# vainaviv/hulk-keypoints

Measured on AMD Instinct MI355X. Metric: images/sec (640x480, N keypoints) inference+train at 1/2/4/8 MI355X, higher is better.
Workload: dtype f32 (f16x3 split-precision MFMA, fp32-accurate); 1 GPU; C2 inference: resnet34-8s K=4 640x480 f16x3 batch 32/GPU (train-mode BN, fused K-ch head, heatmap + argmax, keypoints all-gathered at N>1); mode=infer, backbone=resnet34, keypoints=4, height=480, width=640, batch_per_gpu=32, global_batch=32, parallelism=dp1, bn=per-rank, collectives=none, input=fp32 NCHW (ToTensor)

## Files before the change

### hulk-keypoints_amd/csrc/bn.hip

```cpp
#include <cstdlib>

#include "common.h"

#pragma clang fp contract(off)

namespace hkp {

__device__ __forceinline__ void bn_rank_stats_store(int c, int C, long count, double mean, double m2, double* stats) {
    stats[c] = mean;
    stats[C + c] = m2;
    if (c == 0) stats[2 * C] = (double)count;
}

template <int CPB, int NT = 256, int NB = 0>
__global__ __launch_bounds__(NT) void bn_finalize_kernel(int C, long count, long tiles, int tile_rows,
                                                         const float* __restrict__ part, const float* gamma,
                                                         const float* beta, float momentum, float eps, float* rmean,
                                                         float* rvar, int64_t* nbt, float* ss, float* mi,
                                                         double* stats) {
    constexpr int TL = NT / CPB, NW = NT / 64;
    __shared__ double red[NW][8];
    const int cl = threadIdx.x % CPB, tl = threadIdx.x / CPB, c = blockIdx.x * CPB + cl;
    const bool ok = c < C;
    if constexpr (NB > 0) {
        float2 v[NB];
#pragma unroll
        for (int j = 0; j < NB; ++j) {
            const long t = tl + (long)j * TL;
            v[j] = ok && t < tiles ? *(const float2*)(part + (t * C + c) * 2) : make_float2(0.f, 0.f);
        }
        double s = 0.0;
#pragma unroll
        for (int j = 0; j < NB; ++j) s += (double)v[j].x;
        const double mean = lanes_sum_d<CPB, NW>(s, red) / (double)count;
        const bool pow2 = (tile_rows & (tile_rows - 1)) == 0;
        const double inv_rows = 1.0 / (double)tile_rows;
        double q = 0.0;
#pragma unroll
        for (int j = 0; j < NB; ++j) {
            const long t = tl + (long)j * TL;
            if (ok && t < tiles) {
                const long n_t = min((long)tile_rows, count - t * tile_rows);
                const double tm = pow2 && n_t == tile_rows ? (double)v[j].x * inv_rows : (double)v[j].x / (double)n_t;
                const double dm = tm - mean;
                q += (double)v[j].y + (double)n_t * dm * dm;
            }
        }
        const double m2 = lanes_sum_d<CPB, NW>(q, red);
        if (tl == 0 && ok) {
            if (stats) bn_rank_stats_store(c, C, count, mean, m2, stats);
            else bn_fin_store(c, C, count, mean, m2, gamma, beta, momentum, eps, rmean, rvar, nbt, ss, mi);
        }
        return;
    }
    double s = 0.0;
    if (ok)
        for (long t0 = tl; t0 < tiles; t0 += 8 * TL) {
            float v[8];
#pragma unroll
            for (int j = 0; j < 8; ++j) {
                const long t = t0 + (long)j * TL;
                v[j] = t < tiles ? part[(t * C + c) * 2] : 0.f;
            }
#pragma unroll
            for (int j = 0; j < 8; ++j) s += (double)v[j];
        }
    const double mean = lanes_sum_d<CPB, NW>(s, red) / (double)count;
    double q = 0.0;
    if (ok)
        for (long t0 = tl; t0 < tiles; t0 += 8 * TL) {
            float2 v[8];
#pragma unroll
            for (int j = 0; j < 8; ++j) {
                const long t = t0 + (long)j * TL;
                v[j] = t < tiles ? *(const float2*)(part + (t * C + c) * 2) : make_float2(0.f, 0.f);
            }
#pragma unroll
            for (int j = 0; j < 8; ++j) {
                const long t = t0 + (long)j * TL;
                if (t < tiles) {
                    const long n_t = min((long)tile_rows, count - t * tile_rows);
                    const double dm = (double)v[j].x / (double)n_t - mean;
                    q += (double)v[j].y + (double)n_t * dm * dm;
                }
            }
        }
    const double m2 = lanes_sum_d<CPB, NW>(q, red);
    if (tl == 0 && ok) {
        if (stats) bn_rank_stats_store(c, C, count, mean, m2, stats);
        else bn_fin_store(c, C, count, mean, m2, gamma, beta, momentum, eps, rmean, rvar, nbt, ss, mi);
    }
}

constexpr int FIN_TL = 16, FIN_TPL = 8, FIN_CHUNK = FIN_TL * FIN_TPL;

__device__ __forceinline__ double fin_col_sum(double v, double (*red)[64], int tl, int cl) {
    __syncthreads();
    red[tl][cl] = v;
    __syncthreads();
    double a[FIN_TL];
#pragma unroll
    for (int i = 0; i < FIN_TL; ++i) a[i] = red[i][cl];
#pragma unroll
    for (int w = FIN_TL / 2; w >= 1; w >>= 1)
#pragma unroll
        for (int i = 0; i < w; ++i) a[i] = a[2 * i] + a[2 * i + 1];
    return a[0];
}

__global__ __launch_bounds__(1024) void bn_fin_chunk_kernel(int C, long count, long tiles, int tile_rows,
                                                            const float* __restrict__ part, double2* __restrict__ ws) {
    __shared__ double red[FIN_TL][64];
    const int cl = threadIdx.x & 63, tl = threadIdx.x >> 6, c = blockIdx.x * 64 + cl;
    const bool ok = c < C;
    const long t0 = (long)blockIdx.y * FIN_CHUNK;
    float2 v[FIN_TPL];
#pragma unroll
    for (int j = 0; j < FIN_TPL; ++j) {
        const long t = t0 + tl + (long)FIN_TL * j;
        v[j] = ok && t < tiles ? *(const float2*)(part + (t * C + c) * 2) : make_float2(0.f, 0.f);
    }
    double s = 0.0;
#pragma unroll
    for (int j = 0; j < FIN_TPL; ++j) s += (double)v[j].x;
    const double S = fin_col_sum(s, red, tl, cl);
    const long te = min(tiles, t0 + FIN_CHUNK);
    const long nk = min(count, te * (long)tile_rows) - t0 * (long)tile_rows;
    const double mk = S / (double)nk;
    double q = 0.0;
#pragma unroll
    for (int j = 0; j < FIN_TPL; ++j) {
        const long t = t0 + tl + (long)FIN_TL * j;
        if (t < tiles) {
            const long n_t = min((long)tile_rows, count - t * tile_rows);
            const double dm = (double)v[j].x / (double)n_t - mk;
            q += (double)v[j].y + (double)n_t * dm * dm;
        }
    }
    const double Q = fin_col_sum(q, red, tl, cl);
    if (tl == 0 && ok) ws[blockIdx.y * (long)C + c] = make_double2(S, Q);
}

__global__ __launch_bounds__(1024) void bn_fin_merge_kernel(int C, long count, long chunks, int tile_rows,
                                                            const double2* __restrict__ ws, const float* gamma,
                                                            const float* beta, float momentum, float eps,
                                                            float* rmean, float* rvar, int64_t* nbt, float* ss,
                                                            float* mi, double* stats) {
    __shared__ double red[FIN_TL][64];
    const int cl = threadIdx.x & 63, tl = threadIdx.x >> 6, c = blockIdx.x * 64 + cl;
    const bool ok = c < C;
    const long rows = (long)FIN_CHUNK * tile_rows;
    double s = 0.0;
    if (ok)
        for (long k = tl; k < chunks; k += FIN_TL) s += ws[k * C + c].x;
    const double mean = fin_col_sum(s, red, tl, cl) / (double)count;
    double q = 0.0;
    if (ok)
        for (long k = tl; k < chunks; k += FIN_TL) {
            const double2 w = ws[k * C + c];
            const long nk = min(rows, count - k * rows);
            const double dm = w.x / (double)nk - mean;
            q += w.y + (double)nk * dm * dm;
        }
    const double m2 = fin_col_sum(q, red, tl, cl);
    if (tl == 0 && ok) {
        if (stats) bn_rank_stats_store(c, C, count, mean, m2, stats);
        else bn_fin_store(c, C, count, mean, m2, gamma, beta, momentum, eps, rmean, rvar, nbt, ss, mi);
    }
}

__global__ void bn_fin_ranks_kernel(int C, int R, const double* __restrict__ st, const float* gamma, const float* beta,
                                    float momentum, float eps, float* rmean, float* rvar, int64_t* nbt, float* ss,
                                    float* mi) {
    const int c = blockIdx.x * blockDim.x + threadIdx.x;
    if (c >= C) return;
    const long L = 2L * C + 1;
    double n = 0.0, s = 0.0;
    for (int r = 0; r < R; ++r) {
        const double nr = st[r * L + 2 * C];
        n += nr;
        s += nr * st[r * L + c];
    }
    const double mean = R == 1 ? st[c] : s / n;
    double m2 = 0.0;
    for (int r = 0; r < R; ++r) {
        const double nr = st[r * L + 2 * C], dm = st[r * L + c] - mean;
        m2 += st[r * L + C + c] + nr * dm * dm;
    }
    bn_fin_store(c, C, (long)n, mean, m2, gamma, beta, momentum, eps, rmean, rvar, nbt, ss, mi);
}

__global__ void bn_eval_kernel(int C, const float* gamma, const float* beta, const float* rm, const float* rv,
                               float eps, float* ss, float* mi) {
    const int c = blockIdx.x * blockDim.x + threadIdx.x;
    if (c >= C) return;
    const float inv = (float)(1.0 / sqrt((double)rv[c] + (double)eps));
    const float g = gamma ? gamma[c] : 1.f, b = beta ? beta[c] : 0.f;
    const float alpha = __fmul_rn(inv, g);
    ss[c] = alpha;
    ss[C + c] = __fsub_rn(b, __fmul_rn(rm[c], alpha));
    if (mi) {
        mi[c] = rm[c];
        mi[C + c] = inv;
    }
}

template <int RES, bool RELU, bool FIX>
__global__ __launch_bounds__(256) void bn_apply_kernel(long n4, int C4, const f32x4* __restrict__ y,
                                                       const f32x4* __restrict__ sc, const f32x4* __restrict__ sh,
                                                       const f32x4* __restrict__ res, const f32x4* __restrict__ rsc,
                                                       const f32x4* __restrict__ rsh, const _Float16* __restrict__ rsplit,
                                                       f32x4* __restrict__ out, _Float16* __restrict__ osplit,
                                                       int passes) {
    const long stride = (long)gridDim.x * blockDim.x;
    const long i0 = (long)blockIdx.x * blockDim.x + threadIdx.x;
    struct In {
        f32x4 v, r;
        h16x4 h, l;
    };
    auto load = [&](long i) {
        In x;
        x.v = y[i];
        if constexpr (RES == 1 || RES == 2) x.r = res[i];
        if constexpr (RES == 3) {
            const long e0 = i * 4, off = 2 * e0 - (e0 & 31);
            x.h = *(const h16x4*)(rsplit + off);
            x.l = *(const h16x4*)(rsplit + off + 32);
        }
        return x;
    };
    auto one = [&](long i, const In& x, const f32x4& a, const f32x4& b, const f32x4& ra, const f32x4& rb) {
        f32x4 o;
#pragma unroll
        for (int e = 0; e < 4; ++e) o[e] = __fadd_rn(__fmul_rn(x.v[e], a[e]), b[e]);
        if constexpr (RES == 1) {
#pragma unroll
            for (int e = 0; e < 4; ++e) o[e] = __fadd_rn(o[e], x.r[e]);
        } else if constexpr (RES == 2) {
#pragma unroll
            for (int e = 0; e < 4; ++e) o[e] = __fadd_rn(o[e], __fadd_rn(__fmul_rn(x.r[e], ra[e]), rb[e]));
        } else if constexpr (RES == 3) {
#pragma unroll
            for (int e = 0; e < 4; ++e) o[e] = __fadd_rn(o[e], __fadd_rn((float)x.h[e], (float)x.l[e]));
// ... 83 lines not shown
            one(i + stride, v1, r1);
        }
        if (i < n8) {
            h16x8 r0{};
            if constexpr (RES != 0) r0 = res[i];
            one(i, y[i], r0);
        }
    } else {
        for (long i = i0; i < n8; i += stride) {
            load_ss((int)(i % C8) * 8);
            h16x8 r0{};
            if constexpr (RES != 0) r0 = res[i];
            one(i, y[i], r0);
        }
    }
}

template <typename IDX>
__global__ __launch_bounds__(256) void bn_relu_maxpool_kernel(int N, int H, int W, int C, int Ho, int Wo,
                                                             const float* __restrict__ y,
                                                             const float* __restrict__ ss,
                                                             float* __restrict__ out, _Float16* __restrict__ osplit,
                                                             int passes, uchar4* __restrict__ route) {
    const IDX C4 = (IDX)(C >> 2);
    const IDX total = (IDX)N * (IDX)Ho * (IDX)Wo * C4;
    const IDX stride = (IDX)gridDim.x * (IDX)blockDim.x;
    for (IDX i = (IDX)blockIdx.x * (IDX)blockDim.x + (IDX)threadIdx.x; i < total; i += stride) {
        const int c4 = (int)(i % C4);
        IDX p = i / C4;
        const int wo = (int)(p % (IDX)Wo);
        p /= (IDX)Wo;
        const int ho = (int)(p % (IDX)Ho);
        const int n = (int)(p / (IDX)Ho);
        const f32x4 a = *(const f32x4*)(ss + 4 * c4), b = *(const f32x4*)(ss + C + 4 * c4);
        f32x4 m = {-INFINITY, -INFINITY, -INFINITY, -INFINITY};
        int tap[4] = {0, 0, 0, 0};
#pragma unroll
        for (int dr = 0; dr < 3; ++dr) {
            const int hi = ho * 2 - 1 + dr;
            if ((unsigned)hi >= (unsigned)H) continue;
#pragma unroll
            for (int ds = 0; ds < 3; ++ds) {
                const int wi = wo * 2 - 1 + ds;
                if ((unsigned)wi >= (unsigned)W) continue;
                const f32x4 v = *(const f32x4*)(y + (((long)n * H + hi) * W + wi) * C + 4 * c4);
#pragma unroll
                for (int e = 0; e < 4; ++e) {
                    float t = __fadd_rn(__fmul_rn(v[e], a[e]), b[e]);
                    t = t > 0.f ? t : 0.f;
                    if (t > m[e]) {
                        m[e] = t;
                        tap[e] = dr * 3 + ds;
                    }
                }
            }
        }
        if (out) *(f32x4*)(out + (long)i * 4) = m;
        if (osplit) store_split4(m, (long)i, osplit, passes);
        if (route)
            route[i] = make_uchar4(m[0] > 0.f ? tap[0] : 255, m[1] > 0.f ? tap[1] : 255,
                                   m[2] > 0.f ? tap[2] : 255, m[3] > 0.f ? tap[3] : 255);
    }
}

static inline int grid_for(long work, int block = 256, long cap = 256L * 16) {
    long g = (work + block - 1) / block;
    if (g > cap) g = cap;
    return (int)(g < 1 ? 1 : g);
}

}

using namespace hkp;

HKP_AB_KNOB(int, g_fin_regs, 1);
#ifdef HKP_AB_KNOBS
extern "C" void hkp_debug_fin_regs(int32_t on) { g_fin_regs = on != 0; }
#endif
int hkp_fin_regs() { return g_fin_regs; }

static int fin_one(const char* who, int32_t c, int64_t count, int64_t tiles, int32_t tile_rows, const float* partials,
                   const float* gamma, const float* beta, float momentum, float eps, float* running_mean,
                   float* running_var, int64_t* num_batches_tracked, float* scale_shift, float* mean_invstd,
                   double* stats, hkp_stream_t stream) {
    HKP_CHECK_ARG(c > 0 && count > 0 && tiles > 0 && tile_rows > 0, "%s: bad sizes", who);
    HKP_CHECK_ARG(partials && (scale_shift || stats), "%s: null tensor", who);
    HKP_CHECK_ARG((running_mean == nullptr) == (running_var == nullptr), "%s: running stats pair", who);
    HKP_CHECK_ARG((tiles - 1) * (int64_t)tile_rows < count && tiles * (int64_t)tile_rows >= count,
                  "%s: tiles/tile_rows inconsistent with count", who);
    const int cpb = partials_cpb(c);
    const long per = g_fin_regs ? (tiles + 256 / cpb - 1) / (256 / cpb) : 1L << 40;
#define HKP_FIN1(CPB, NT, NB)                                                                                      \
    hipLaunchKernelGGL((bn_finalize_kernel<CPB, NT, NB>), dim3((c + CPB - 1) / CPB), dim3(NT), 0, as_stream(stream), \
                       c, (long)count, (long)tiles, tile_rows, partials, gamma, beta, momentum, eps, running_mean,   \
                       running_var, num_batches_tracked, scale_shift, mean_invstd, stats)
#define HKP_FIN(CPB)                                  \
    if (tiles >= 4096) { HKP_FIN1(CPB, 1024, 0); } \
    else if (per <= 8) { HKP_FIN1(CPB, 256, 8); } \
    else if (per <= 16) { HKP_FIN1(CPB, 256, 16); } \
    else if (per <= 32) { HKP_FIN1(CPB, 256, 32); } \
    else { HKP_FIN1(CPB, 256, 0); }
    if (cpb == 8) { HKP_FIN(8); }
    else if (cpb == 4) { HKP_FIN(4); }
    else if (cpb == 2) { HKP_FIN(2); }
    else { HKP_FIN(1); }
#undef HKP_FIN
#undef HKP_FIN1
    HKP_LAUNCH_CHECK(who);
    return HKP_OK;
}

extern "C" int64_t hkp_bn_finalize_workspace_bytes(int32_t c, int64_t tiles) {
    if (c <= 0 || tiles <= 0) return -1;
    return ((tiles + FIN_CHUNK - 1) / FIN_CHUNK) * (int64_t)c * (int64_t)sizeof(double2);
}

static int fin_two(const char* who, int32_t c, int64_t count, int64_t tiles, int32_t tile_rows, const float* partials,
                   const float* gamma, const float* beta, float momentum, float eps, float* running_mean,
                   float* running_var, int64_t* num_batches_tracked, float* scale_shift, float* mean_invstd,
                   double* stats, void* workspace, int64_t ws_bytes, hkp_stream_t stream) {
    HKP_CHECK_ARG(c > 0 && count > 0 && tiles > 0 && tile_rows > 0, "%s: bad sizes", who);
    HKP_CHECK_ARG(partials && (scale_shift || stats) && workspace, "%s: null tensor", who);
    HKP_CHECK_ARG((running_mean == nullptr) == (running_var == nullptr), "%s: running stats pair", who);
    HKP_CHECK_ARG((tiles - 1) * (int64_t)tile_rows < count && tiles * (int64_t)tile_rows >= count,
                  "%s: tiles/tile_rows inconsistent with count", who);
    const int64_t need = hkp_bn_finalize_workspace_bytes(c, tiles);
    HKP_CHECK_ARG(ws_bytes >= need, "%s: workspace %ld < %ld", who, (long)ws_bytes, (long)need);
    const long chunks = (tiles + FIN_CHUNK - 1) / FIN_CHUNK;
    hipStream_t st = as_stream(stream);
    const unsigned cg = (unsigned)((c + 63) / 64);
    hipLaunchKernelGGL(bn_fin_chunk_kernel, dim3(cg, (unsigned)chunks), dim3(1024), 0, st, c, (long)count,
                       (long)tiles, tile_rows, partials, (double2*)workspace);
    HKP_LAUNCH_CHECK(who);
    hipLaunchKernelGGL(bn_fin_merge_kernel, dim3(cg), dim3(1024), 0, st, c, (long)count, chunks, tile_rows,
                       (const double2*)workspace, gamma, beta, momentum, eps, running_mean, running_var,
                       num_batches_tracked, scale_shift, mean_invstd, stats);
    HKP_LAUNCH_CHECK(who);
    return HKP_OK;
}

extern "C" int hkp_bn_finalize(int32_t c, int64_t count, int64_t tiles, int32_t tile_rows, const float* partials,
                               const float* gamma, const float* beta, float momentum, float eps, float* running_mean,
                               float* running_var, int64_t* num_batches_tracked, float* scale_shift,
                               float* mean_invstd, hkp_stream_t stream) {
    HKP_CHECK_ARG(scale_shift, "hkp_bn_finalize: null tensor");
    return fin_one("hkp_bn_finalize", c, count, tiles, tile_rows, partials, gamma, beta, momentum, eps, running_mean,
                   running_var, num_batches_tracked, scale_shift, mean_invstd, nullptr, stream);
}

extern "C" int hkp_bn_finalize_ws(int32_t c, int64_t count, int64_t tiles, int32_t tile_rows, const float* partials,
                                  const float* gamma, const float* beta, float momentum, float eps,
                                  float* running_mean, float* running_var, int64_t* num_batches_tracked,
                                  float* scale_shift, float* mean_invstd, void* workspace, int64_t ws_bytes,
                                  hkp_stream_t stream) {
    HKP_CHECK_ARG(scale_shift, "hkp_bn_finalize_ws: null tensor");
    return fin_two("hkp_bn_finalize_ws", c, count, tiles, tile_rows, partials, gamma, beta, momentum, eps,
                   running_mean, running_var, num_batches_tracked, scale_shift, mean_invstd, nullptr, workspace,
                   ws_bytes, stream);
}

extern "C" int hkp_bn_stats(int32_t c, int64_t count, int64_t tiles, int32_t tile_rows, const float* partials,
                            double* stats, void* workspace, int64_t ws_bytes, hkp_stream_t stream) {
    HKP_CHECK_ARG(stats, "hkp_bn_stats: null tensor");
    if (workspace)
        return fin_two("hkp_bn_stats", c, count, tiles, tile_rows, partials, nullptr, nullptr, 0.f, 0.f, nullptr,
                       nullptr, nullptr, nullptr, nullptr, stats, workspace, ws_bytes, stream);
    return fin_one("hkp_bn_stats", c, count, tiles, tile_rows, partials, nullptr, nullptr, 0.f, 0.f, nullptr, nullptr,
                   nullptr, nullptr, nullptr, stats, stream);
}

extern "C" int hkp_bn_finalize_ranks(int32_t c, int32_t nranks, const double* stats, const float* gamma,
                                     const float* beta, float momentum, float eps, float* running_mean,
                                     float* running_var, int64_t* num_batches_tracked, float* scale_shift,
                                     float* mean_invstd, hkp_stream_t stream) {
    HKP_CHECK_ARG(c > 0 && nranks > 0, "hkp_bn_finalize_ranks: bad sizes");
    HKP_CHECK_ARG(stats && scale_shift, "hkp_bn_finalize_ranks: null tensor");
    HKP_CHECK_ARG((running_mean == nullptr) == (running_var == nullptr), "hkp_bn_finalize_ranks: running stats pair");
    hipLaunchKernelGGL(bn_fin_ranks_kernel, dim3((c + 255) / 256), dim3(256), 0, as_stream(stream), c, nranks, stats,
                       gamma, beta, momentum, eps, running_mean, running_var, num_batches_tracked, scale_shift,
                       mean_invstd);
    HKP_LAUNCH_CHECK("hkp_bn_finalize_ranks");
    return HKP_OK;
}

extern "C" int hkp_bn_eval_params(int32_t c, const float* gamma, const float* beta, const float* running_mean,
                                  const float* running_var, float eps, float* scale_shift, float* mean_invstd,
                                  hkp_stream_t stream) {
    HKP_CHECK_ARG(c > 0 && running_mean && running_var && scale_shift, "hkp_bn_eval_params: bad args");
    hipLaunchKernelGGL(bn_eval_kernel, dim3((c + 255) / 256), dim3(256), 0, as_stream(stream), c, gamma, beta,
                       running_mean, running_var, eps, scale_shift, mean_invstd);
    HKP_LAUNCH_CHECK("hkp_bn_eval_params");
    return HKP_OK;
}

extern "C" int hkp_bn_apply(int64_t m, int32_t c, const float* y, const float* scale_shift, const float* res,
                            const float* res_scale_shift, const uint16_t* res_split, int32_t relu, float* out,
                            uint16_t* out_split, int32_t split_passes, hkp_stream_t stream) {
    HKP_CHECK_ARG(m > 0 && c > 0 && c % 4 == 0, "hkp_bn_apply: need m>0 and c%%4==0 (c=%d)", c);
    HKP_CHECK_ARG(y && scale_shift && (out || out_split), "hkp_bn_apply: null tensor");
    HKP_CHECK_ARG(!out_split || ((split_passes == 1 || split_passes == 3) && c % 32 == 0),
                  "hkp_bn_apply: split output needs split_passes 1|3 and c%%32==0");
    HKP_CHECK_ARG(res_scale_shift == nullptr || res != nullptr, "hkp_bn_apply: res_scale_shift without res");
    HKP_CHECK_ARG(res_split == nullptr || (res == nullptr && c % 32 == 0),
                  "hkp_bn_apply: res_split excludes res and needs c%%32==0");
    const long n4 = m * (long)c / 4;
    const int C4 = c / 4;
    const f32x4 *Y = (const f32x4*)y, *SC = (const f32x4*)scale_shift, *SH = (const f32x4*)(scale_shift + c);
    const f32x4* R = (const f32x4*)res;
    const f32x4* RSC = res_scale_shift ? (const f32x4*)res_scale_shift : nullptr;
    const f32x4* RSH = res_scale_shift ? (const f32x4*)(res_scale_shift + c) : nullptr;
    f32x4* O = (f32x4*)out;
    const int g = grid_for(n4);
    hipStream_t st = as_stream(stream);
    const bool fix = ((long)g * 256) % C4 == 0;
#define HKP_APPLY(RES, RL)                                                                                         \
    if (fix)                                                                                                       \
        hipLaunchKernelGGL((bn_apply_kernel<RES, RL, true>), dim3(g), dim3(256), 0, st, n4, C4, Y, SC, SH, R, RSC, \
                           RSH, (const _Float16*)res_split, O, (_Float16*)out_split, split_passes);               \
    else                                                                                                           \
        hipLaunchKernelGGL((bn_apply_kernel<RES, RL, false>), dim3(g), dim3(256), 0, st, n4, C4, Y, SC, SH, R,     \
                           RSC, RSH, (const _Float16*)res_split, O, (_Float16*)out_split, split_passes)
    if (res_split) {
        if (relu) HKP_APPLY(3, true); else HKP_APPLY(3, false);
    } else if (!res) {
        if (relu) HKP_APPLY(0, true); else HKP_APPLY(0, false);
    } else if (!res_scale_shift) {
        if (relu) HKP_APPLY(1, true); else HKP_APPLY(1, false);
    } else {
        if (relu) HKP_APPLY(2, true); else HKP_APPLY(2, false);
    }
#undef HKP_APPLY
    HKP_LAUNCH_CHECK("hkp_bn_apply");
    return HKP_OK;
}

extern "C" int hkp_bn_relu_maxpool(int32_t n, int32_t h, int32_t w, int32_t c, const float* y,
                                   const float* scale_shift, float* out, uint16_t* out_split,
                                   int32_t split_passes, uint8_t* route, hkp_stream_t stream) {
    HKP_CHECK_ARG(n > 0 && h > 0 && w > 0 && c > 0 && c % 4 == 0, "hkp_bn_relu_maxpool: bad sizes");
    HKP_CHECK_ARG(y && scale_shift && (out || out_split), "hkp_bn_relu_maxpool: null tensor");
    HKP_CHECK_ARG(!out_split || ((split_passes == 1 || split_passes == 3) && c % 32 == 0),
                  "hkp_bn_relu_maxpool: split output needs split_passes 1|3 and c%%32==0");
    const int ho = (h - 1) / 2 + 1, wo = (w - 1) / 2 + 1;
    const long work = (long)n * ho * wo * (c / 4);
    const bool idx32 = work * 4 < (1L << 31) && (long)n * h * w * c < (1L << 31);
    if (idx32)
        hipLaunchKernelGGL(bn_relu_maxpool_kernel<unsigned>, dim3(grid_for(work)), dim3(256), 0, as_stream(stream), n,
                           h, w, c, ho, wo, y, scale_shift, out, (_Float16*)out_split, split_passes, (uchar4*)route);
    else
        hipLaunchKernelGGL(bn_relu_maxpool_kernel<long>, dim3(grid_for(work)), dim3(256), 0, as_stream(stream), n, h,
                           w, c, ho, wo, y, scale_shift, out, (_Float16*)out_split, split_passes, (uchar4*)route);
// ... 35 lines not shown
```

### hulk-keypoints_amd/csrc/conv_x3.hip

```cpp
#include <algorithm>
#include <cstdlib>
#include <type_traits>

#include "common.h"

namespace hkp {

typedef _Float16 f16x8 __attribute__((ext_vector_type(8)));

__device__ __attribute__((aligned(256))) uint4 g_x3_zero_line[8];
__device__ __attribute__((aligned(256))) uint4 g_x3_nan_line[8] = {
    {~0u, ~0u, ~0u, ~0u}, {~0u, ~0u, ~0u, ~0u}, {~0u, ~0u, ~0u, ~0u}, {~0u, ~0u, ~0u, ~0u},
    {~0u, ~0u, ~0u, ~0u}, {~0u, ~0u, ~0u, ~0u}, {~0u, ~0u, ~0u, ~0u}, {~0u, ~0u, ~0u, ~0u}};

struct X3Args {
    const _Float16* xs;
    const _Float16* ws;
    const float* wscale;
    float* y;
    _Float16* y16 = nullptr;
    float* part;
    const unsigned* amax;
    const float* add;
    int N, H, W, C, K, R, S, stride, pad, dil, Ho, Wo;
    int M, nks, cch, n_tiles, RS;
    long plane;
    int ost = 0, OH = 0, OW = 0, oy = 0, ox = 0;
    int mt0 = 0;
    long sk_units = 0;
    float* sk_ws = nullptr;
    unsigned* sk_cnt = nullptr;
    int sk_grid = 0, sk_b = 0;
    int sk_one = 0;
    int main_blocks = 0, tail_groups = 0, tail_mt0 = 0;
    long tail_units = 0;
    unsigned long long* stamps = nullptr;
    int stagger_blocks = 0, stagger_ticks = 0;
    const float* ep_ss = nullptr;
    const _Float16* ep_res = nullptr;
    const float* ep_rss = nullptr;
    int ep_relu = 0;
    const float* in_ss = nullptr;
    int st_kind = 0;
    int prio = 0;
#ifdef HKP_AB_KNOBS
    int a_wrap = 0;
#endif
};

typedef unsigned x3u32x4 __attribute__((ext_vector_type(4)));
template <typename V>
__device__ __forceinline__ void x3_st16(V* p, const V& val, int kind, int dflt) {
    static_assert(sizeof(V) == 16, "16-B store");
    x3u32x4 v;
    __builtin_memcpy(&v, &val, 16);
    x3u32x4* q = (x3u32x4*)p;
    const int k = kind ? kind : dflt;
    if (k == 2) {
        __builtin_nontemporal_store(v, q);
    } else if (k == 3) {
        asm volatile("global_store_dwordx4 %0, %1, off sc1" ::"v"(q), "v"(v) : "memory");
    } else if (k == 4) {
        asm volatile("global_store_dwordx4 %0, %1, off sc0 sc1" ::"v"(q), "v"(v) : "memory");
    } else {
        *q = v;
    }
}

__device__ __forceinline__ void x3_stamp(const X3Args& a, int k) {
    if (a.stamps && threadIdx.x == 0) a.stamps[blockIdx.x * 8 + k] = __builtin_amdgcn_s_memrealtime();
}
__device__ __forceinline__ void x3_stamp_where(const X3Args& a) {
    if (a.stamps && threadIdx.x == 0) {
        a.stamps[blockIdx.x * 8 + 6] = (unsigned)__builtin_amdgcn_s_getreg((31 << 11) | 4);
        a.stamps[blockIdx.x * 8 + 7] = (unsigned)__builtin_amdgcn_s_getreg((31 << 11) | 20);
    }
}

__device__ __forceinline__ float pow2_scale_of(float m) {
    if (!(m > 0.f) || !(m < INFINITY)) return 1.f;
    int e;
    frexpf(m, &e);
    e = 14 - e;
    e = e < -100 ? -100 : (e > 100 ? 100 : e);
    return ldexpf(1.f, e);
}

__device__ __forceinline__ void lds_barrier() {
    asm volatile("" ::: "memory");
    __builtin_amdgcn_s_barrier();
    asm volatile("" ::: "memory");
}

__device__ __forceinline__ void lds_sync() {
    asm volatile("s_waitcnt lgkmcnt(0)" ::: "memory");
    lds_barrier();
}

__device__ __forceinline__ void glds16(const void* src, char* lds_wave_base) {
    __builtin_amdgcn_global_load_lds(src, (__attribute__((address_space(3))) void*)lds_wave_base, 16, 0, 0);
}

typedef int i32x4 __attribute__((ext_vector_type(4)));
extern "C" __device__ void hkp_raw_buffer_load_lds(i32x4 rsrc, __attribute__((address_space(3))) void* lds, int size,
                                                   int voffset, int soffset, int offset,
                                                   int aux) __asm("llvm.amdgcn.raw.buffer.load.lds");
__device__ __forceinline__ i32x4 buffer_rsrc(const void* base, unsigned bytes) {
    const unsigned long long p = (unsigned long long)base;
    i32x4 r;
    r[0] = __builtin_amdgcn_readfirstlane((int)(unsigned)p);
    r[1] = __builtin_amdgcn_readfirstlane((int)(unsigned)(p >> 32) & 0xFFFF);
// ... 65 lines not shown
        }
        *(volatile int*)flag_lds = last;
    }
    __syncthreads();
    if (!*(volatile int*)flag_lds) return false;
    static_assert(NV4 % 8 == 0 || NV4 < 8, "sk_combine chunks");
    constexpr int CW = NV4 < 8 ? NV4 : 8;
    for (int sg = 0; sg < nseg; ++sg) {
        const gf32x4* p = slab(b0 + sg);
#pragma unroll
        for (int v0 = 0; v0 < NV4; v0 += CW) {
            f32x4 x[CW];
#pragma unroll
            for (int v = 0; v < CW; ++v) x[v] = p[(v0 + v) * 512 + tid];
#pragma unroll
            for (int v = 0; v < CW; ++v) set(v0 + v, sg == 0 ? x[v] : get(v0 + v) + x[v]);
        }
    }
    return true;
}

__device__ __forceinline__ long x3_out_off(const X3Args& a, int m, int n) {
    if (m >= a.M) return -1;
    long pix = m;
    if (a.ost) {
        const int hw = a.Ho * a.Wo, ni = m / hw, rem = m - ni * hw;
        const int ho = rem / a.Wo, wo = rem - ho * a.Wo;
        pix = ((long)ni * a.OH + ho * a.ost + a.oy) * a.OW + wo * a.ost + a.ox;
    }
    return pix * a.K + n;
}

__device__ __forceinline__ void x3_store(const X3Args& a, long off, float v, float av) {
    if (off < 0) return;
    v = a.add ? v + av : v;
    if (a.y16) a.y16[off] = (_Float16)v;
    else a.y[off] = v;
}

constexpr bool x3_packed(int P) { return P != 1; }
constexpr int x3_nprod(int P) { return P == 3 ? 3 : 2; }

template <int P, typename V, typename Acc, typename Mfma>
__device__ __forceinline__ void x3_products(Acc& acc, const V& a0, const V& a1, const V& b0, const V& b1, Mfma&& mfma) {
    if constexpr (P == 3) {
        acc = mfma(a0, b0, acc);
        acc = mfma(a0, b1, acc);
        acc = mfma(a1, b0, acc);
    } else if constexpr (P == 2) {
        acc = mfma(a0, b0, acc);
        acc = mfma(a1, b0, acc);
    } else if constexpr (P == 4) {
        acc = mfma(a0, b0, acc);
        acc = mfma(a0, b1, acc);
    } else {
        acc = mfma(a0, b0, acc);
        acc = mfma(a1, b1, acc);
    }
}

template <int BN, int NI, int NJ, int NR, int CW, int SHF, typename Val, typename Row>
__device__ __forceinline__ void x3_bn_partials(const X3Args& a, char* smem, int m0, int n0, int wm, int wn, int lane,
                                               int tid, Val&& val, Row&& row) {
    constexpr int WM = 4;
    __syncthreads();
    float* red = (float*)smem;
    float* tmean = red + WM * BN;
    float colsum[NJ];
#pragma unroll
    for (int j = 0; j < NJ; ++j) {
        float s = 0.f;
#pragma unroll
        for (int i = 0; i < NI; ++i)
#pragma unroll
            for (int r = 0; r < NR; ++r) s += (row(i, r) < a.M) ? val(i, j, r) : 0.f;
        for (int o = SHF; o < 64; o <<= 1) s += __shfl_xor(s, o);
        colsum[j] = s;
    }
    if (lane < CW) {
#pragma unroll
        for (int j = 0; j < NJ; ++j) red[wm * BN + wn * NJ * CW + j * CW + lane] = colsum[j];
    }
    __syncthreads();
    const long tile128 = (long)(m0 >> 7);
    for (int e = tid; e < 2 * BN; e += 512) {
        const int h = e / BN, c = e - h * BN;
        const int cnt = min(128, a.M - (m0 + 128 * h));
        if (cnt > 0) {
            const float s = red[(2 * h) * BN + c] + red[(2 * h + 1) * BN + c];
            tmean[h * BN + c] = s / (float)cnt;
            a.part[((tile128 + h) * a.K + n0 + c) * 2 + 0] = s;
        }
    }
    __syncthreads();
    const float* mu_h = tmean + (wm >> 1) * BN;
#pragma unroll
    for (int j = 0; j < NJ; ++j) {
        const float mu = mu_h[wn * NJ * CW + j * CW + (lane % CW)];
        float q = 0.f;
#pragma unroll
        for (int i = 0; i < NI; ++i)
#pragma unroll
            for (int r = 0; r < NR; ++r) {
                const float d = val(i, j, r) - mu;
                q += (row(i, r) < a.M) ? d * d : 0.f;
            }
        for (int o = SHF; o < 64; o <<= 1) q += __shfl_xor(q, o);
        colsum[j] = q;
    }
    __syncthreads();
    if (lane < CW) {
#pragma unroll
        for (int j = 0; j < NJ; ++j) red[wm * BN + wn * NJ * CW + j * CW + lane] = colsum[j];
    }
    __syncthreads();
    for (int e = tid; e < 2 * BN; e += 512) {
        const int h = e / BN, c = e - h * BN;
        if (a.M - (m0 + 128 * h) > 0)
            a.part[((tile128 + h) * a.K + n0 + c) * 2 + 1] = red[(2 * h) * BN + c] + red[(2 * h + 1) * BN + c];
    }
}

__device__ __forceinline__ void x3_chan_merge(float& s, float& q, float s2, float q2, float inv_n, float f) {
    const float d = s2 * inv_n - s * inv_n;
    s = s + s2;
    q = (q + q2) + d * d * f;
}

template <int BN, int NI, int NJ, int CW, int SHF, int WMP = 4, typename Vec, typename Row, typename Sc>
__device__ __forceinline__ void x3_bn_partials_w(const X3Args& a, float* red, int m0, int n0, int wm, int wn,
                                                 int lane, Vec&& vec, Row&& row, Sc&& sc_of,
                                                 float* wide = nullptr) {
    constexpr int WROWS = 16 * NI;
    if constexpr (CW == 16 && SHF == 16 && WMP == 4 && (NI == 4 || NI == 3)) {
        if (wide != nullptr && m0 + 4 * WROWS <= a.M) {
            const int q = lane >> 4, r16 = lane & 15;
            constexpr float inv = 1.f / (NI * 4);
            float ls[NJ], lq[NJ];
#pragma unroll
            for (int j = 0; j < NJ; ++j) {
                f32x4 s4 = vec(0, j);
#pragma unroll
                for (int i = 1; i < NI; ++i) s4 += vec(i, j);
                const float s = (s4[0] + s4[1]) + (s4[2] + s4[3]);
                const f32x4 mu = {s * inv, s * inv, s * inv, s * inv};
                f32x4 q4 = {0.f, 0.f, 0.f, 0.f};
#pragma unroll
                for (int i = 0; i < NI; ++i) {
                    const f32x4 d = vec(i, j) - mu;
                    q4 += d * d;
                }
                ls[j] = s;
                lq[j] = (q4[0] + q4[1]) + (q4[2] + q4[3]);
            }
            lds_sync();
#pragma unroll
            for (int j = 0; j < NJ; ++j) {
                const int c = wn * NJ * CW + j * CW + r16;
                wide[(wm * 4 + q) * BN + c] = ls[j];
                wide[16 * BN + (wm * 4 + q) * BN + c] = lq[j];
                if (wm == 0 && q == 0) wide[32 * BN + c] = sc_of(j);
            }
            lds_sync();
            for (int t = threadIdx.x; t < 2 * BN; t += blockDim.x) {
                const int h = t / BN, c = t - h * BN;
                float S[2], Q[2];
#pragma unroll
                for (int v = 0; v < 2; ++v) {
                    const int w4 = (2 * h + v) * 4;
                    float s[4], qq[4];
#pragma unroll
                    for (int g = 0; g < 4; ++g) {
                        s[g] = wide[(w4 + g) * BN + c];
                        qq[g] = wide[16 * BN + (w4 + g) * BN + c];
                    }
                    constexpr float n1 = 4.f * NI;
                    x3_chan_merge(s[0], qq[0], s[1], qq[1], 1.f / n1, n1 / 2);
                    x3_chan_merge(s[2], qq[2], s[3], qq[3], 1.f / n1, n1 / 2);
                    x3_chan_merge(s[0], qq[0], s[2], qq[2], 1.f / (2 * n1), n1);
                    S[v] = s[0];
                    Q[v] = qq[0];
                }
                x3_chan_merge(S[0], Q[0], S[1], Q[1], 1.f / (16 * NI), 8.f * NI);
                const float sc = wide[32 * BN + c];
                const long tile128 = (long)(m0 / (2 * WROWS)) + h;
                a.part[(tile128 * a.K + n0 + c) * 2 + 0] = S[0] * sc;
                a.part[(tile128 * a.K + n0 + c) * 2 + 1] = Q[0] * (sc * sc);
            }
            return;
        }
    }
    float* rs = red;
    float* rq = red + 4 * BN;
    const int nw = min(WROWS, max(0, a.M - (m0 + WROWS * wm)));
    float ls[NJ], lq[NJ], ln;
    if (nw == WROWS) {
        ln = (float)(NI * 4);
        constexpr float inv = 1.f / (NI * 4);
#pragma unroll
        for (int j = 0; j < NJ; ++j) {
            f32x4 s4 = vec(0, j);
#pragma unroll
            for (int i = 1; i < NI; ++i) s4 += vec(i, j);
            const float s = (s4[0] + s4[1]) + (s4[2] + s4[3]);
            const f32x4 mu = {s * inv, s * inv, s * inv, s * inv};
            f32x4 q4 = {0.f, 0.f, 0.f, 0.f};
#pragma unroll
            for (int i = 0; i < NI; ++i) {
                const f32x4 d = vec(i, j) - mu;
                q4 += d * d;
            }
            ls[j] = s;
            lq[j] = (q4[0] + q4[1]) + (q4[2] + q4[3]);
        }
    } else {
        ln = 0.f;
#pragma unroll
        for (int i = 0; i < NI; ++i)
#pragma unroll
            for (int r = 0; r < 4; ++r) ln += (row(i, r) < a.M) ? 1.f : 0.f;
        const float linv = ln > 0.f ? 1.f / ln : 0.f;
#pragma unroll
        for (int j = 0; j < NJ; ++j) {
            float s = 0.f;
#pragma unroll
            for (int i = 0; i < NI; ++i)
#pragma unroll
                for (int r = 0; r < 4; ++r) s += (row(i, r) < a.M) ? vec(i, j)[r] : 0.f;
            const float mu = s * linv;
            float q = 0.f;
#pragma unroll
            for (int i = 0; i < NI; ++i)
#pragma unroll
                for (int r = 0; r < 4; ++r) {
                    const float d = vec(i, j)[r] - mu;
                    q += (row(i, r) < a.M) ? d * d : 0.f;
                }
            ls[j] = s;
            lq[j] = q;
        }
    }
    for (int o = SHF; o < 64; o <<= 1) {
        const float nb = __shfl_xor(ln, o);
        const float nt = ln + nb;
        const float f = nt > 0.f ? ln * nb / nt : 0.f;
        const float ia = ln > 0.f ? 1.f / ln : 0.f, ib = nb > 0.f ? 1.f / nb : 0.f;
#pragma unroll
        for (int j = 0; j < NJ; ++j) {
            const float sb = __shfl_xor(ls[j], o), qb = __shfl_xor(lq[j], o);
            const float d = sb * ib - ls[j] * ia;
            ls[j] = ls[j] + sb;
            lq[j] = (lq[j] + qb) + d * d * f;
        }
        ln = nt;
    }
    if constexpr (WMP == 2) {
        if (nw == 0 || lane >= CW) return;
        const long pt = (long)(m0 / WROWS) + wm;
#pragma unroll
        for (int j = 0; j < NJ; ++j) {
            const int c = wn * NJ * CW + j * CW + lane;
            const float sc = sc_of(j);
            a.part[(pt * a.K + n0 + c) * 2 + 0] = ls[j] * sc;
            a.part[(pt * a.K + n0 + c) * 2 + 1] = lq[j] * (sc * sc);
        }
        return;
    }
    if (lane < CW) {
#pragma unroll
        for (int j = 0; j < NJ; ++j) {
            const int c = wn * NJ * CW + j * CW + lane;
            rs[wm * BN + c] = ls[j];
            rq[wm * BN + c] = lq[j];
        }
    }
    lds_sync();
    const int nb = min(WROWS, max(0, a.M - (m0 + WROWS * (wm | 1))));
    if ((wm & 1) || nw == 0 || lane >= CW) return;
    const long tile128 = (long)(m0 / (2 * WROWS)) + (wm >> 1);
    const float ia = 1.f / (float)nw, ib = nb > 0 ? 1.f / (float)nb : 0.f;
    const float f = (float)nw * (float)nb / (float)(nw + nb);
#pragma unroll
    for (int j = 0; j < NJ; ++j) {
        const int c = wn * NJ * CW + j * CW + lane;
        const float sa = rs[wm * BN + c], qa = rq[wm * BN + c];
        const float sb = rs[(wm + 1) * BN + c], qb = rq[(wm + 1) * BN + c];
        const float d = sb * ib - sa * ia;
        const float sum = nb > 0 ? sa + sb : sa;
        const float m2 = nb > 0 ? (qa + qb) + d * d * f : qa;
        const float sc = sc_of(j);
        a.part[(tile128 * a.K + n0 + c) * 2 + 0] = sum * sc;
        a.part[(tile128 * a.K + n0 + c) * 2 + 1] = m2 * (sc * sc);
    }
}

template <int BN>
__device__ __forceinline__ void x3_store_tile_f16(const X3Args& a, const char* smem, int m0, int n0, int tid) {
    constexpr int CH = BN / 8, PITCH = BN + 8;
#pragma unroll 4
    for (int e = tid; e < 256 * CH; e += 512) {
        const int row = e / CH, cc = e - row * CH;
        const int m = m0 + row;
        if (m < a.M)
            x3_st16((uint4*)(a.y16 + (long)m * a.K + n0 + cc * 8), *(const uint4*)(smem + (row * PITCH + cc * 8) * 2), a.st_kind, 1);
    }
}

template <int BN>
struct X3Res {
    static constexpr int NPT = 256 * (BN / 8) / 512;
    f16x8 r[NPT];
};
template <int BN>
__device__ __forceinline__ X3Res<BN> x3_ep_res_load(const X3Args& a, int m0, int n0, int tid) {
    constexpr int CH = BN / 8;
    X3Res<BN> res;
    const int cc = tid % CH;
#pragma unroll
    for (int u = 0; u < X3Res<BN>::NPT; ++u) {
        const int row = (tid + 512 * u) / CH, m = m0 + row;
        res.r[u] = f16x8{};
        if (a.ep_res && m < a.M)
            res.r[u] = __builtin_nontemporal_load((const f16x8*)(a.ep_res + (long)m * a.K + n0 + cc * 8));
    }
    return res;
}

template <int BN>
__device__ __forceinline__ void x3_store_tile_f16_bn(const X3Args& a, const char* smem, const float* ssl,
                                                     const X3Res<BN>& res, int m0, int n0, int tid) {
    constexpr int CH = BN / 8, PITCH = BN + 8;
    static_assert(512 % CH == 0, "fixed channels per thread");
    const int cc = tid % CH;
    float sa[8], sb[8], ra[8], rb[8];
#pragma unroll
    for (int e = 0; e < 8; ++e) {
        sa[e] = ssl[cc * 8 + e];
        sb[e] = ssl[BN + cc * 8 + e];
        ra[e] = ssl[2 * BN + cc * 8 + e];
        rb[e] = ssl[3 * BN + cc * 8 + e];
    }
    const bool hres = a.ep_res != nullptr, rsc = a.ep_rss != nullptr, relu = a.ep_relu != 0;
#pragma unroll
    for (int u = 0; u < X3Res<BN>::NPT; ++u) {
        const int row = (tid + 512 * u) / CH;
        const int m = m0 + row;
        if (m >= a.M) continue;
        const long off = (long)m * a.K + n0 + cc * 8;
        const f16x8 v = *(const f16x8*)(smem + (row * PITCH + cc * 8) * 2);
        const f16x8 r = res.r[u];
        f16x8 h;
#pragma unroll
        for (int k = 0; k < 8; ++k) {
            float o = __fadd_rn(__fmul_rn((float)v[k], sa[k]), sb[k]);
            if (hres) o = rsc ? __fadd_rn(o, __fadd_rn(__fmul_rn((float)r[k], ra[k]), rb[k])) : __fadd_rn(o, (float)r[k]);
            if (relu) o = o > 0.f ? o : 0.f;
            h[k] = (_Float16)o;
        }
        x3_st16((f16x8*)(a.y16 + off), h, a.st_kind, 2);
    }
}

// ... 285 lines not shown
#pragma unroll
    for (int j = 0; j < UN; ++j) sc[j] = col_scale(wn * UN * 16 + j * 16 + r16);
    if (a.part) {
        if constexpr (RINGSCR) lds_sync();
        x3_bn_partials_w<BN, UM, UN, 16, 16, WM>(
            a, (float*)(smem + RED_OFF), m0, n0, wm, wn, lane, [&](int i, int j) { return acc[i][j]; },
            [&](int i, int r) { return rbase + i * 16 + r; }, [&](int j) { return sc[j]; }, (float*)smem);
    }
    x3_stamp(a, 3);
    {
        constexpr int PASSES = BN == 256 ? 2 : 1, RPP = BM / PASSES, PITCH = BN + 4, C4 = BN / 4;
        static_assert(RPP * PITCH * 4 <= LDS_ALL, "staging");
        float* t = (float*)smem;
        lds_sync();
#pragma unroll
        for (int h = 0; h < PASSES; ++h) {
            if (PASSES == 1 || (wm * UM * 16) / RPP == h) {
#pragma unroll
                for (int i = 0; i < UM; ++i)
#pragma unroll
                    for (int j = 0; j < UN; ++j)
#pragma unroll
                        for (int r = 0; r < 4; ++r)
                            t[(wm * UM * 16 + i * 16 + 4 * q + r - h * RPP) * PITCH + wn * UN * 16 + j * 16 + r16] =
                                acc[i][j][r] * sc[j];
            }
            lds_sync();
            if (!a.add && !a.ost) {
#pragma unroll 4
                for (int e = tid; e < RPP * C4; e += 512) {
                    const int row = e / C4, c4 = e - row * C4;
                    const int m = m0 + h * RPP + row;
                    if (m < a.M)
                        x3_st16((f32x4*)(a.y + (long)m * a.K + n0 + c4 * 4), *(const f32x4*)(t + row * PITCH + c4 * 4),
                                a.st_kind, 2);
                }
            } else {
#pragma unroll 2
                for (int e = tid; e < RPP * C4; e += 512) {
                    const int row = e / C4, c4 = e - row * C4;
                    const long off = x3_out_off(a, m0 + h * RPP + row, n0 + c4 * 4);
                    if (off >= 0) {
                        f32x4 v = *(const f32x4*)(t + row * PITCH + c4 * 4);
                        if (a.add) {
                            const f32x4 ad = *(const f32x4*)(a.add + off);
#pragma unroll
                            for (int k = 0; k < 4; ++k) v[k] = v[k] + ad[k];
                        }
                        *(f32x4*)(a.y + off) = v;
                    }
                }
            }
            if (h + 1 < PASSES) lds_sync();
        }
    }
    x3_stamp(a, 4);
    x3_stamp(a, 5);
}

template <int BN, bool STEM, bool PAIR, int MFD, int P, bool A3 = false, int BM = 256>
__device__ __forceinline__ void conv_x3_tile(const X3Args& a, char* smem, int tile, int ks, int nks, bool partial) {
    constexpr int WM = x3_wm(BM), WN = 8 / WM;
    constexpr int TM = BM / (WM * 32), TN = BN / (WN * 32);
    constexpr int ROW = 128;
    constexpr int CPR = ROW / 16;
    constexpr int RPI = 1024 / ROW;
    constexpr int NST = x3_nst(BN, PAIR);
    constexpr int STAGE = (BM + BN) * ROW;
    constexpr int GA = (BM / RPI + 7) / 8;
    constexpr bool A_SINK = BM / RPI % 8 != 0;
    constexpr int GBT = BN / RPI;
    constexpr int GB = GBT >= 8 ? GBT / 8 : 1;
    constexpr int GL = GA + GB;
    static_assert(MFD == 16 || MFD == 32, "bad conv_x3 MFMA shape");
    static_assert(P == 3 || ((P == 1 || P == 2 || P == 4) && !STEM), "bad conv_x3 operand layout");
    static_assert(!(MFD == 32 && BN == 256), "256x256 tiles run the 16x16x32 body");
    static_assert(NST * STAGE <= 160 * 1024, "LDS");
    static_assert(!A3 || ((BN == 256 || (BN == 128 && BM == 160)) && !STEM && !PAIR && MFD == 16),
                  "A3: the 16x16x32 body on 256-wide tiles (128-wide: 160 rows)");
    static_assert(BM == 256 || (A3 && (BM == 192 || BM == 160) && x3_packed(P)), "192- / 160-row tiles: A3, packed");
    static_assert(!A_SINK || A3, "the A sink is the A3 body's");

    const int mt = tile / a.n_tiles, nt = tile - mt * a.n_tiles;
    const int m0 = (mt + a.mt0) * BM, n0 = nt * BN;
    const int tid = threadIdx.x, lane = tid & 63;
    const int w = __builtin_amdgcn_readfirstlane(tid >> 6);
    const int wm = w / WN, wn = w % WN;

    auto swz = [](int row) { return (row >> 1) & 7; };
    auto lofs = [&](int L) -> long {
        if constexpr (STEM) return (L >> 2) * a.plane + (L & 3) * 8;
        else return L * 8;
    };

    const int cstride = STEM ? 4 : a.cch * 64;
    const long xbias = (long)a.pad * (a.W + 1) * cstride;
    const _Float16* xbase = a.xs - xbias;
    int a_org[GA];
    unsigned a_off[GA];
#pragma unroll
    for (int i = 0; i < GA; ++i) {
        const int row = RPI * (w * GA + i) + lane / CPR;
        const int Lc = (lane % CPR) ^ swz(row);
        const long L = lofs(Lc);
#ifdef HKP_AB_KNOBS
        const int m = a.a_wrap ? (m0 + row) % a.a_wrap : m0 + row;
#else
        const int m = m0 + row;
#endif
        int hb = -16384, wb = -16384;
        long off = 0;
        if (m < a.M && (!A_SINK || RPI * (w * GA + i) < BM)) {
            const int hw = a.Ho * a.Wo;
            const int n = m / hw, rem = m - n * hw;
            const int ho = rem / a.Wo, wo = rem - ho * a.Wo;
            hb = ho * a.stride - a.pad;
            wb = wo * a.stride - a.pad;
            off = (((long)n * a.H + hb) * a.W + wb) * cstride + L;
        }
        a_org[i] = (int)(((unsigned)hb << 16) | ((unsigned)wb & 0xFFFFu));
        a_off[i] = (unsigned)(off + xbias);
    }
    const int bline = a.RS * a.cch * 64;
    int b_off[GB], b_dst[GB];
#pragma unroll
    for (int j = 0; j < GB; ++j) {
        const int bi = (w * GB + j) % GBT;
        const int row = RPI * bi + lane / CPR;
        const int Lc = (lane % CPR) ^ swz(row);
        b_off[j] = (n0 + row) * bline + (STEM ? Lc * 8 : (int)lofs(Lc));
        b_dst[j] = (BM + RPI * bi) * ROW;
    }
    const _Float16* zero = (const _Float16*)g_x3_zero_line;

    int q_buf = 0;
    int q_cc = ks / a.RS;
    int q_tap = ks - q_cc * a.RS;
    int q_rr = q_tap / a.S, q_ss = q_tap - q_rr * a.S;
    auto issue_next = [&]() {
        char* st = smem + q_buf * STAGE;
        const int dh = q_rr * a.dil, dw = q_ss * a.dil;
        const long toff = ((long)dh * a.W + dw) * cstride + q_cc * 64;
#pragma unroll
        for (int i = 0; i < GA; ++i) {
            const int hb = a_org[i] >> 16, wb = (int)(short)(a_org[i] & 0xFFFF);
            const bool in = (unsigned)(hb + dh) < (unsigned)a.H && (unsigned)(wb + dw) < (unsigned)a.W;
            glds16(in ? xbase + ((unsigned long)a_off[i] + toff) : zero, st + (RPI * (w * GA + i)) * ROW);
        }
        const int boff = (q_tap * a.cch + q_cc) * 64;
#pragma unroll
        for (int j = 0; j < GB; ++j) glds16(a.ws + (unsigned)(b_off[j] + boff), st + b_dst[j]);
        q_buf = q_buf == NST - 1 ? 0 : q_buf + 1;
        if (++q_ss == a.S) {
            q_ss = 0;
            ++q_rr;
        }
        if (++q_tap == a.RS) {
            q_tap = 0;
            q_rr = 0;
            ++q_cc;
        }
    };

    int qa_buf = 0, qa_cc = q_cc, qa_tap = q_tap, qa_rr = q_rr, qa_ss = q_ss;
    int qb_buf = 0, qb_cc = q_cc, qb_tap = q_tap;
    auto issue_a = [&]() {
        {
// ... 194 lines not shown
        [&](int i, int r) { return rbase + i * 32 + (r & 3) + 8 * (r >> 2); });
    }
}

__device__ __forceinline__ void x3_stagger(const X3Args& a) {
    const int b = blockIdx.x;
    if (a.stagger_ticks > 0 && b < a.stagger_blocks && ((b >> 3) & 1)) {
        const unsigned long long t0 = __builtin_amdgcn_s_memrealtime();
        while (__builtin_amdgcn_s_memrealtime() - t0 < (unsigned long long)a.stagger_ticks) __builtin_amdgcn_s_sleep(2);
    }
}

template <int BN, bool STEM, bool PAIR, int MFD, bool SK, int P>
__global__ __launch_bounds__(512, PAIR ? 2 : 1) void conv_x3_kernel(X3Args a) {
    __shared__ __attribute__((aligned(1024))) char smem[x3_lds_bytes(BN, PAIR, P) + x3_red_bytes(BN, PAIR)];
    if constexpr (!SK) x3_stagger(a);
    x3_stamp(a, 0);
    const int G = gridDim.x, b = xcd_remap(blockIdx.x, G);
    if constexpr (!SK) {
        conv_x3_tile<BN, STEM, PAIR, MFD, P>(a, smem, b, 0, a.nks, false);
        return;
    }
    const int NT = a.n_tiles, NG = G / NT, g = b / NT, nt = b - g * NT;
    if (g >= NG) return;
    const long U = a.sk_units, u0 = sk_start(g, U, NG), u1 = sk_start(g + 1, U, NG);
    for (long u = u0; u < u1;) {
        const int mt = (int)(u / a.nks);
        const long t0 = (long)mt * a.nks;
        const int ks = (int)(u - t0), ke = (int)min((long)a.nks, u1 - t0);
        if (u != u0) __syncthreads();
        conv_x3_tile<BN, STEM, PAIR, MFD, P>(a, smem, mt * NT + nt, ks, ke - ks, ks != 0 || ke != a.nks);
        u = t0 + ke;
    }
}

template <int P>
__device__ __forceinline__ void conv_x3_a3_grid(const X3Args& a, char* smem) {
    x3_stagger(a);
    x3_stamp(a, 0);
    const int b = blockIdx.x;
    if (a.tail_groups == 0 || b < a.main_blocks) {
        conv_x3_tile<256, false, false, 16, P, true>(
            a, smem, xcd_remap(b, a.tail_groups ? a.main_blocks : gridDim.x), 0, a.nks, false);
        return;
    }
    X3Args t = a;
    const int NT = a.n_tiles, G = a.tail_groups * NT;
    t.mt0 = a.tail_mt0;
    t.sk_units = a.tail_units;
    t.sk_grid = G;
    t.sk_b = xcd_remap(b - a.main_blocks, G);
    const int g = t.sk_b / NT, nt = t.sk_b - g * NT;
    const long U = t.sk_units, u0 = sk_start(g, U, a.tail_groups), u1 = sk_start(g + 1, U, a.tail_groups);
    const int mt = (int)(u0 / a.nks);
    const int ks = (int)(u0 - (long)mt * a.nks), ke = (int)(u1 - (long)mt * a.nks);
    conv_x3_tile<256, false, false, 16, P, true>(t, smem, mt * NT + nt, ks, ke - ks, true);
}

template <int P>
__global__ __launch_bounds__(512, 1) void conv_x3_a3_kernel(X3Args a) {
    __shared__ __attribute__((aligned(1024))) char smem[X3_A3_LDS];
    conv_x3_a3_grid<P>(a, smem);
}

template <int P>
__global__ __launch_bounds__(512, 1) void conv_x3_a3_192_kernel(X3Args a) {
    __shared__ __attribute__((aligned(1024))) char smem[x3_a3_lds(192)];
    x3_stamp(a, 0);
    conv_x3_tile<256, false, false, 16, P, true, 192>(a, smem, xcd_remap(blockIdx.x, gridDim.x), 0, a.nks, false);
}

template <int P>
__global__ __launch_bounds__(512, 1) void conv_x3_a3_160_kernel(X3Args a) {
    __shared__ __attribute__((aligned(1024))) char smem[x3_a3_lds(160)];
    x3_stamp(a, 0);
    conv_x3_tile<256, false, false, 16, P, true, 160>(a, smem, xcd_remap(blockIdx.x, gridDim.x), 0, a.nks, false);
}

template <int P>
__global__ __launch_bounds__(512, 1) void conv_x3_a3_160x128_kernel(X3Args a) {
    __shared__ __attribute__((aligned(1024))) char smem[x3_a3_lds(160, 128)];
    x3_stamp(a, 0);
    conv_x3_tile<128, false, false, 16, P, true, 160>(a, smem, xcd_remap(blockIdx.x, gridDim.x), 0, a.nks, false);
}

template <int BN, int P>
__global__ __launch_bounds__(512, 1) void conv_x3_tail_kernel(X3Args a) {
    __shared__ __attribute__((aligned(1024))) char smem[x3_lds_bytes(BN, false, P) + x3_red_bytes(BN, false)];
    const int G = gridDim.x, b = xcd_remap(blockIdx.x, G);
    const int NT = a.n_tiles, NG = G / NT, g = b / NT, nt = b - g * NT;
    const long U = a.sk_units, u0 = sk_start(g, U, NG), u1 = sk_start(g + 1, U, NG);
    const int mt = (int)(u0 / a.nks);
    const int ks = (int)(u0 - (long)mt * a.nks), ke = (int)(u1 - (long)mt * a.nks);
    conv_x3_tile<BN, false, false, 16, P>(a, smem, mt * NT + nt, ks, ke - ks, true);
}

constexpr int HALO_PH = 8, HALO_PW = 32, HALO_LW = HALO_PW + 2, HALO_NL = (HALO_PH + 2) * HALO_LW;
constexpr int HALO_GA = 6;
constexpr int HALO_ABYTES = 8 * HALO_GA * 8 * 128;
constexpr int HALO_NSTB = 3, HALO_BSTAGE = 64 * 128;
constexpr int HALO_LDS = HALO_ABYTES + HALO_NSTB * HALO_BSTAGE;

__device__ __forceinline__ int halo_swz(int L) { return L & 6; }

static bool halo_shape(int stride, int r, int s, int pad, int dil, int ho, int wo, int k) {
    return stride == 1 && r == 3 && s == 3 && pad == 1 && dil == 1 && ho % HALO_PH == 0 && wo % HALO_PW == 0 &&
           k % 64 == 0;
}

template <int P, bool BNIN>
__device__ __forceinline__ void x3_halo_bnin(const X3Args& a, char* smem, int g, int tid) {
    constexpr int ROW = 128;
    constexpr int PIECES = P == 1 ? 8 : 4;
    constexpr int LPI = 512 / PIECES;
    constexpr int NL = 8 * HALO_GA * 8;
    const int j = tid % PIECES;
    const int c0 = g * (P == 1 ? 64 : 32) + 8 * j;
    float sa[8], sb[8];
#pragma unroll
    for (int e = 0; e < 8; ++e) {
        sa[e] = a.in_ss[c0 + e];
        sb[e] = a.in_ss[a.C + c0 + e];
    }
#pragma unroll
    for (int L0 = 0; L0 < NL; L0 += LPI) {
        const int L = L0 + tid / PIECES;
        const int sw = halo_swz(L);
        char* line = smem + L * ROW;
        if constexpr (P == 1) {
            f16x8* ch = (f16x8*)(line + ((j ^ sw) << 4));
            const f16x8 v = *ch;
            f16x8 o;
#pragma unroll
            for (int e = 0; e < 8; ++e) {
                float x = __fadd_rn(__fmul_rn((float)v[e], sa[e]), sb[e]);
                o[e] = (_Float16)(x > 0.f ? x : 0.f);
            }
            *ch = o;
        } else {
            const f32x4 v0 = *(const f32x4*)(line + (((2 * j) ^ sw) << 4));
            const f32x4 v1 = *(const f32x4*)(line + (((2 * j + 1) ^ sw) << 4));
            f16x8 h, l;
#pragma unroll
            for (int e = 0; e < 8; ++e) {
                const float y = e < 4 ? v0[e] : v1[e - 4];
                float x = __fadd_rn(__fmul_rn(y, sa[e]), sb[e]);
                x = x > 0.f ? x : 0.f;
                const _Float16 hv = (_Float16)x;
                h[e] = hv;
                l[e] = (_Float16)(x - (float)hv);
            }
            *(f16x8*)(line + ((j ^ sw) << 4)) = h;
            *(f16x8*)(line + (((4 + j) ^ sw) << 4)) = l;
        }
    }
}

template <int P, bool BNIN>
__device__ __forceinline__ void conv_x3_halo_body(const X3Args& a, char* smem) {
    constexpr int BM = 256, BN = 64, WM = 4, WN = 2, ROW = 128;
    constexpr int UM = BM / (WM * 16), UN = BN / (WN * 16);
    static_assert(256 * (BN + 4) * 4 <= HALO_LDS && 8 * BN * 4 <= HALO_LDS, "epilogue staging");
    static_assert(!BNIN || P == 3 || P == 1, "fused input BN: f16x3 or plain fp16");

    const int tile = xcd_remap(blockIdx.x, gridDim.x);
    const int mt = tile / a.n_tiles, nt = tile - mt * a.n_tiles;
// ... 1466 lines not shown
        const int c = e & 3, s = (e >> 2) & 7, r = e >> 5;
        const float v = (s < 7 && c < C) ? wk[(c * 7 + r) * 7 + s] * sc : 0.f;
        split_store(v, out + ((long)k * 7 + r) * 64 + s * 4 + c);
    }
    if (threadIdx.x == 0) wscale[k] = 1.f / sc;
}

static bool stem_x3_shape(const hkp_conv_desc* d) {
    return d && d->in_layout == HKP_LAYOUT_NCHW && d->c >= 1 && d->c <= 4 && d->r == 7 && d->s == 7 &&
           d->stride == 2 && d->pad == 3 && d->dilation == 1 && d->k % 64 == 0;
}

static int x3_cus() {
    static int n = [] {
        int dev = 0, v = 0;
        if (hipGetDevice(&dev) != hipSuccess || hipDeviceGetAttribute(&v, hipDeviceAttributeMultiprocessorCount, dev) !=
                                                      hipSuccess || v <= 0)
            v = 256;
        return v;
    }();
    return n;
}

constexpr long X3_SK_CNT_BYTES = 64 << 10;
static long x3_sk_ws_bytes(int bn) { return X3_SK_CNT_BYTES + 2L * x3_cus() * bn * 1024; }

static double sk_over(int nks) { return 0.2 + 19.0 / nks; }

HKP_AB_KNOB(int, g_x3_split_tail, 0);
static long x3_tail_groups(long m_tiles, int nt, int nks, double* cost = nullptr) {
    const long G = x3_cus(), tiles = m_tiles * nt, tr = tiles % G;
    const long tm = m_tiles - tiles / G * G / nt;
    double best = 1.0;
    long ng = 0;
    if (tr > 0) {
        for (int S = 2; S <= 8 && nks / S >= 4 && tm * S * nt <= G; ++S)
            if (1.0 / S + 0.08 < best - 1e-9) {
                best = 1.0 / S + 0.08;
                ng = tm * S;
            }
    }
    if (cost) *cost = tr > 0 ? best : 0.0;
    return ng;
}

struct X3Plan {
    int bn;
    bool sk;
};
static X3Plan x3_plan(int k, long m_tiles, int nks, bool sk_ok, double over) {
    const int G = x3_cus();
    X3Plan best{64, false};
    double best_cost = 1e300;
    for (int bn : {256, 128, 64}) {
        if (k % bn) continue;
        const long tiles = m_tiles * (k / bn);
        const double col = bn * (bn == 256 ? 0.9 : bn == 128 ? 1.0 : 1.25);
        double tail = (tiles % G) ? 1.0 : 0.0;
        if (bn == 256 && sk_ok) x3_tail_groups(m_tiles, k / bn, nks, &tail);
        const double dp = ((double)(tiles / G) + tail) * col;
        if (dp < best_cost - 1e-9) {
            best_cost = dp;
            best = {bn, false};
        }
        const int ng = G / (k / bn);
        if (sk_ok && bn != 256 && ng > 0 && m_tiles % ng && tiles * 4 <= X3_SK_CNT_BYTES) {
            const double skc = ((double)m_tiles / ng + over) * col;
            if (skc < best_cost - 1e-9) {
                best_cost = skc;
                best = {bn, true};
            }
        }
    }
    return best;
}

struct X3Choice {
    int bn, mfd;
    bool pair, sk;
    bool halo = false;
    bool a3 = false;
    bool duo = false;
    int bm = 256;
};
static X3Choice x3_choose_base(int k, long m_tiles, int nks, bool sk_ok, int policy, int halo);
static X3Choice x3_choose(int k, long m_tiles, int nks, bool sk_ok, int policy, int halo, int P);
HKP_AB_KNOB(int, g_x3_pair128, 1);
static X3Choice x3_choose(int k, long m_tiles, int nks, bool sk_ok, int policy, int halo, int P) {
    if (policy == HKP_TILE_DUO) {
        if (P == 1 && k % DUO_BN == 0) {
            X3Choice c{DUO_BN, 16, false, false};
            c.duo = true;
            return c;
        }
        policy = HKP_TILE_AUTO;
    }
    if (policy == HKP_TILE_256_A3 && P == 3 && k % 256 != 0 && g_x3_pair128) policy = HKP_TILE_AUTO;
    if (policy == HKP_TILE_192_A3 && (!x3_packed(P) || k % 256 != 0)) policy = HKP_TILE_AUTO;
    if (policy == HKP_TILE_160_A3 && (!x3_packed(P) || k % 128 != 0)) policy = HKP_TILE_AUTO;
    if (policy != HKP_TILE_AUTO_A3 && policy != HKP_TILE_AUTO) return x3_choose_base(k, m_tiles, nks, sk_ok, policy, halo);
    X3Choice c = x3_choose_base(k, m_tiles, nks, sk_ok, HKP_TILE_AUTO, halo);
    if (c.bn == 256 && !c.sk && !c.halo && !c.pair) c.a3 = true;
    if (policy == HKP_TILE_AUTO && P == 1 && !c.halo && k % DUO_BN == 0 && (nks == 1 || k == DUO_BN)) {
        X3Choice d{DUO_BN, 16, false, false};
        d.duo = true;
        return d;
    }
    if (policy == HKP_TILE_AUTO && P == 3 && !c.halo && !c.sk && g_x3_pair128) {
        const bool small = (double)m_tiles * k <= 3.0 * 256 * x3_cus();
        if (small && (nks <= 8 || (c.bn == 128 && m_tiles * (k / 128) >= x3_cus()))) return {64, 16, true, false};
        if (c.bn == 128 && m_tiles * (k / 128) < x3_cus()) c.mfd = 16;
    }
    return c;
}
static X3Choice x3_choose_base(int k, long m_tiles, int nks, bool sk_ok, int policy, int halo) {
    if ((halo >= 1 && policy == HKP_TILE_HALO) ||
        (halo == 2 && (policy == HKP_TILE_AUTO || policy == HKP_TILE_256_TAIL || policy == HKP_TILE_256_A3 ||
                       policy == HKP_TILE_192_A3 || policy == HKP_TILE_160_A3))) {
        X3Choice c{64, 16, true, false};
        c.halo = true;
        return c;
    }
    switch (policy) {
        case HKP_TILE_256:
            if (k % 256 == 0) return {256, 16, false, false};
            break;
        case HKP_TILE_128_MF16:
            if (k % 128 == 0) return {128, 16, false, false};
            break;
        case HKP_TILE_128_MF32:
            if (k % 128 == 0) return {128, 32, false, false};
            break;
        case HKP_TILE_64_PAIR:
            return {64, 16, true, false};
        case HKP_TILE_256_TAIL:
            if (k % 256 == 0) return {256, 16, false, false};
            break;
        case HKP_TILE_256_A3:
            if (k % 256 == 0) return {256, 16, false, false, false, true};
            break;
        case HKP_TILE_192_A3:
        case HKP_TILE_160_A3:
            if (k % 256 == 0 || (policy == HKP_TILE_160_A3 && k % 128 == 0)) {
                X3Choice c{k % 256 == 0 ? 256 : 128, 16, false, false, false, true};
                c.bm = policy == HKP_TILE_192_A3 ? 192 : 160;
                return c;
            }
            break;
        default:
            break;
    }
    const bool sk = sk_ok && policy != HKP_TILE_NO_SK && policy != HKP_TILE_256_TAIL && policy != HKP_TILE_256_A3;
    const X3Plan pl = x3_plan(k, m_tiles, nks, sk, policy == HKP_TILE_SK ? 0.0 : sk_over(nks));
    if (pl.sk) return {pl.bn, pl.bn == 128 ? 16 : 32, false, true};
    if (pl.bn == 256) return {256, 16, false, false};
    if (pl.bn == 128) return {128, (double)m_tiles * (k / 128) >= 2.0 * x3_cus() ? 16 : 32, false, false};
    return {64, 16, true, false};
}

static const X3Choice X3_STEM{64, 16, true, false};

static int x3_kernel_name(const X3Choice& c, bool stem, int P, char* buf, int len) {
    if (c.halo) return snprintf(buf, len, "conv_x3_halo_kernel<%d>", P);
    if (c.duo) return snprintf(buf, len, "conv_x3_duo_kernel<%d>", P);
    if (c.a3)
        return snprintf(buf, len, c.bm == 192                  ? "conv_x3_a3_192_kernel<%d>"
                                  : c.bm == 160 && c.bn == 128 ? "conv_x3_a3_160x128_kernel<%d>"
                                  : c.bm == 160                ? "conv_x3_a3_160_kernel<%d>"
                                                               : "conv_x3_a3_kernel<%d>", P);
    return snprintf(buf, len, "conv_x3_kernel<%d, %s, %s, %d, %s, %d>", c.bn, stem ? "true" : "false",
                    c.pair ? "true" : "false", c.mfd, c.sk ? "true" : "false", P);
}

template <int P>
static void launch_a3(dim3 grid, hipStream_t st, const X3Args& a) {
    hipLaunchKernelGGL(conv_x3_a3_kernel<P>, grid, dim3(512), 0, st, a);
}

template <int P>
static void launch_x3_p(const X3Choice& c, dim3 grid, hipStream_t st, const X3Args& a) {
    if (c.a3)
        launch_a3<P>(grid, st, a);
    else if (c.sk && c.bn == 128)
        hipLaunchKernelGGL((conv_x3_kernel<128, false, false, 16, true, P>), grid, dim3(512), 0, st, a);
    else if (c.sk)
        hipLaunchKernelGGL((conv_x3_kernel<64, false, false, 32, true, P>), grid, dim3(512), 0, st, a);
    else if (c.bn == 256)
        hipLaunchKernelGGL((conv_x3_kernel<256, false, false, 16, false, P>), grid, dim3(512), 0, st, a);
    else if (c.bn == 128 && c.mfd == 16)
        hipLaunchKernelGGL((conv_x3_kernel<128, false, false, 16, false, P>), grid, dim3(512), 0, st, a);
    else if (c.bn == 128)
        hipLaunchKernelGGL((conv_x3_kernel<128, false, false, 32, false, P>), grid, dim3(512), 0, st, a);
    else
        hipLaunchKernelGGL((conv_x3_kernel<64, false, true, 16, false, P>), grid, dim3(512), 0, st, a);
}

HKP_AB_KNOB(unsigned long long*, g_x3_stamps, nullptr);
HKP_AB_KNOB(int, g_x3_stagger_ns, 0);
HKP_AB_KNOB(int, g_x3_store, 0);
HKP_AB_KNOB(int, g_duo_stagger_ns, -1);
HKP_AB_KNOB(int, g_x3_prio, 0);
HKP_AB_KNOB(int, g_x3_a_wrap, 0);

static int x3_halo_level(bool ok, int lines, int P) {
    return !ok ? 0 : lines * (x3_packed(P) ? 32 : 64) <= 64 ? 2 : 1;
}

static bool x3_halo_ok(const X3Args& a, int k) {
    return halo_shape(a.stride, a.R, a.S, a.pad, a.dil, a.Ho, a.Wo, k) && a.ost == 0 && a.ep_ss == nullptr &&
           a.mt0 == 0 && a.plane == 0 && (long)a.N * a.H * a.W * a.cch * 64L + 64 < (1L << 32);
}

template <typename F>
static void x3_dispatch_p(int P, F&& f) {
    switch (P) {
        case 3: f(std::integral_constant<int, 3>{}); break;
        case 1: f(std::integral_constant<int, 1>{}); break;
        case 2: f(std::integral_constant<int, 2>{}); break;
        case 4: f(std::integral_constant<int, 4>{}); break;
        default: break;
    }
}

static void launch_x3(int k, long m_tiles, int policy, int P, hipStream_t st, X3Args& a, void* ws = nullptr,
                      int64_t ws_bytes = 0) {
    a.stamps = g_x3_stamps;
    a.st_kind = g_x3_store;
    a.prio = g_x3_prio;
#ifdef HKP_AB_KNOBS
    a.a_wrap = g_x3_a_wrap;
#endif
    a.stagger_ticks = g_x3_stagger_ns / 10;
    a.stagger_blocks = x3_cus();
    const bool sk_ok = ws && ws_bytes >= x3_sk_ws_bytes(256);
    const int nks = a.RS * a.cch;
    const X3Choice c = x3_choose(k, m_tiles, nks, sk_ok, policy, x3_halo_level(x3_halo_ok(a, k), a.cch, P), P);
    a.n_tiles = k / c.bn;
    a.nks = nks;
    a.sk_units = 0;
    if (c.duo) {
        const long blocks = m_tiles * a.n_tiles;
        const int ns = g_duo_stagger_ns < 0 ? 5500 + 450 * 2 * nks : g_duo_stagger_ns;
        a.stagger_ticks = blocks > 2L * x3_cus() ? ns / 10 : 0;
        a.stagger_blocks = 2 * x3_cus();
        hipLaunchKernelGGL(conv_x3_duo_kernel<1>, dim3((unsigned)blocks), dim3(256), 0, st, a);
        return;
    }
    if (c.halo) {
        const dim3 gh((unsigned)(m_tiles * a.n_tiles));
        if (a.in_ss) {
            if (P == 3) hipLaunchKernelGGL(conv_x3_halo_bnin_kernel<3>, gh, dim3(512), 0, st, a);
            else hipLaunchKernelGGL(conv_x3_halo_bnin_kernel<1>, gh, dim3(512), 0, st, a);
        } else {
            x3_dispatch_p(P, [&](auto pc) { hipLaunchKernelGGL(conv_x3_halo_kernel<pc.value>, gh, dim3(512), 0, st, a); });
        }
        return;
    }
    if (c.bm != 256) {
        const long mt = ((long)a.M + c.bm - 1) / c.bm;
        const dim3 gm((unsigned)(mt * a.n_tiles));
        x3_dispatch_p(P, [&](auto pc) {
            if constexpr (x3_packed(pc.value)) {
                if (c.bm == 192) hipLaunchKernelGGL(conv_x3_a3_192_kernel<pc.value>, gm, dim3(512), 0, st, a);
                else if (c.bn == 128) hipLaunchKernelGGL(conv_x3_a3_160x128_kernel<pc.value>, gm, dim3(512), 0, st, a);
                else hipLaunchKernelGGL(conv_x3_a3_160_kernel<pc.value>, gm, dim3(512), 0, st, a);
            }
        });
        return;
    }
    dim3 grid((unsigned)(m_tiles * a.n_tiles));
    if (c.sk) {
        a.sk_units = m_tiles * a.nks;
        a.sk_cnt = (unsigned*)ws;
        a.sk_ws = (float*)((char*)ws + X3_SK_CNT_BYTES);
        const long ng = std::min<long>(x3_cus() / a.n_tiles, a.sk_units);
        grid = dim3((unsigned)(ng * a.n_tiles));
    }
    const long tiles = m_tiles * a.n_tiles;
    const long G = x3_cus();
    const long rm = tiles / G * G / a.n_tiles;
    const long tm = m_tiles - rm;
    long NG = (!c.sk && c.bn == 256 && sk_ok &&
               (policy == HKP_TILE_AUTO || policy == HKP_TILE_256_TAIL || policy == HKP_TILE_256_A3 ||
                policy == HKP_TILE_AUTO_A3))
                  ? x3_tail_groups(m_tiles, a.n_tiles, nks)
                  : 0;
    if (NG > 0 && !(tm > 0 && NG % tm == 0 && NG * a.n_tiles <= G && tm * nks >= NG &&
                    NG * a.n_tiles * 256L * 1024 + X3_SK_CNT_BYTES <= ws_bytes && tm * a.n_tiles * 4 <= X3_SK_CNT_BYTES))
        NG = 0;
    const bool tail = NG > 0;
    a.sk_one = tail;
    if (tail && c.a3 && !g_x3_split_tail) {
        X3Args t = a;
        t.main_blocks = (int)(rm * a.n_tiles);
        t.tail_groups = (int)NG;
        t.tail_mt0 = (int)rm;
        t.tail_units = tm * nks;
        t.sk_cnt = (unsigned*)ws;
        t.sk_ws = (float*)((char*)ws + X3_SK_CNT_BYTES);
        const dim3 g1((unsigned)((rm + NG) * a.n_tiles));
        x3_dispatch_p(P, [&](auto pc) { launch_a3<pc.value>(g1, st, t); });
        return;
    }
    if (tail) {
        if (rm > 0) {
            dim3 g0((unsigned)(rm * a.n_tiles));
            x3_dispatch_p(P, [&](auto pc) { launch_x3_p<pc.value>(c, g0, st, a); });
        }
        X3Args t = a;
        t.mt0 = (int)rm;
        t.sk_units = tm * nks;
        t.sk_cnt = (unsigned*)ws;
        t.sk_ws = (float*)((char*)ws + X3_SK_CNT_BYTES);
        const dim3 gt((unsigned)(NG * a.n_tiles));
        x3_dispatch_p(P, [&](auto pc) { hipLaunchKernelGGL((conv_x3_tail_kernel<256, pc.value>), gt, dim3(512), 0, st, t); });
        return;
    }
    x3_dispatch_p(P, [&](auto pc) { launch_x3_p<pc.value>(c, grid, st, a); });
}

}

using namespace hkp;

extern "C" int hkp_weight_pack_x3(int32_t k, int32_t rsc, int32_t c, const float* w, uint16_t* w_split,
                                  float* w_inv_scale, hkp_stream_t stream) {
    HKP_CHECK_ARG(k > 0 && c > 0 && c % 32 == 0 && rsc > 0 && rsc % c == 0 && w && w_split && w_inv_scale,
                  "hkp_weight_pack_x3: bad args");
    hipLaunchKernelGGL(weight_pack_x3_kernel, dim3(k), dim3(256), 0, as_stream(stream), rsc, w, (_Float16*)w_split,
                       w_inv_scale);
    HKP_LAUNCH_CHECK("hkp_weight_pack_x3");
    return HKP_OK;
}

extern "C" int hkp_weight_pack_f16(int32_t k, int32_t rsc, const float* w, uint16_t* w_f16, float* w_inv_scale,
                                   hkp_stream_t stream) {
    HKP_CHECK_ARG(k > 0 && rsc > 0 && w && w_f16 && w_inv_scale, "hkp_weight_pack_f16: bad args");
    hipLaunchKernelGGL(weight_pack_f16_kernel, dim3(k), dim3(256), 0, as_stream(stream), rsc, w, (_Float16*)w_f16,
                       w_inv_scale);
    HKP_LAUNCH_CHECK("hkp_weight_pack_f16");
    return HKP_OK;
}

extern "C" int64_t hkp_conv_x3_sk_workspace_bytes(void) { return x3_sk_ws_bytes(256); }

static bool x3_offsets_fit(long n, long h, long w, long cstride, long k, long rs) {
    return (n * h * w + 64 * (w + 65)) * cstride < (1L << 32) && k * rs * cstride < (1L << 31);
}

static int check_tile(const hkp_conv_desc* d, const char* who) {
    HKP_CHECK_ARG(d->tile >= HKP_TILE_AUTO && d->tile <= HKP_TILE_160_A3, "%s: unknown tile policy %d", who,
                  d->tile);
    HKP_CHECK_ARG(d->tile != HKP_TILE_RESERVED_7 && d->tile != HKP_TILE_RESERVED_8 && d->tile != HKP_TILE_RESERVED_14,
                  "%s: tile policy %d is retired (a persistent conv body, measured slower)", who, d->tile);
    return HKP_OK;
}

static int conv_fwd_x3_common(const hkp_conv_desc* d, const uint16_t* xs, const uint16_t* ws, const float* wsc,
                              float* y, uint16_t* y16, float* part, void* sk_ws, int64_t sk_bytes, int P,
                              hkp_stream_t stream, const char* who, const X3Args* ep = nullptr) {
    int ho, wo;
    int rc = hkp_conv_out_hw(d, &ho, &wo);
    if (rc) return rc;
    rc = check_tile(d, who);
    if (rc) return rc;
    HKP_CHECK_ARG(xs && ws && (x3_packed(P) ? y != nullptr && y16 == nullptr : y == nullptr && y16 != nullptr),
                  "%s: null tensor (the packed split writes fp32 y, P 1 fp16 y)", who);
    HKP_CHECK_ARG(d->in_layout == HKP_LAYOUT_NHWC, "%s: NHWC only", who);
    const int cg = x3_packed(P) ? 32 : 64;
    HKP_CHECK_ARG(d->c % cg == 0 && d->k % 64 == 0, "%s: need Cin%%%d==0, Cout%%64==0 (c=%d k=%d)", who, cg, d->c,
                  d->k);
    const long M = (long)d->n * ho * wo;
    HKP_CHECK_ARG(M < (1L << 31) && x3_offsets_fit(d->n, d->h, d->w, d->c / cg * 64, d->k, d->r * d->s), "%s: too large",
                  who);
    X3Args a;
    a.xs = (const _Float16*)xs; a.ws = (const _Float16*)ws; a.wscale = wsc;
    a.y = y; a.y16 = (_Float16*)y16; a.part = part; a.amax = nullptr; a.add = nullptr; a.plane = 0;
    a.N = d->n; a.H = d->h; a.W = d->w; a.C = d->c; a.K = d->k; a.R = d->r; a.S = d->s;
    a.stride = d->stride; a.pad = d->pad; a.dil = d->dilation; a.Ho = ho; a.Wo = wo;
    a.M = (int)M; a.cch = d->c / cg; a.RS = d->r * d->s;
    int policy = d->tile;
    if (ep) {
        a.ep_ss = ep->ep_ss; a.ep_res = ep->ep_res; a.ep_rss = ep->ep_rss; a.ep_relu = ep->ep_relu;
        a.in_ss = ep->in_ss;
    }
    if (a.in_ss) {
        HKP_CHECK_ARG(P == 3 || P == 1, "%s: fused input BN needs f16x3 or plain fp16", who);
        const bool sk_ok = sk_ws && sk_bytes >= x3_sk_ws_bytes(256);
        const X3Choice c = x3_choose(d->k, (M + 255) / 256, a.RS * a.cch, sk_ok, d->tile,
                                     x3_halo_level(x3_halo_ok(a, d->k), a.cch, P), P);
        HKP_CHECK_ARG(c.halo,
                      "%s: the fused input BN needs a launch on the halo-tile body (stride-1 3x3, pad = dil = 1, "
                      "Ho %% 8 == 0, Wo %% 32 == 0)", who);
    }
    launch_x3(d->k, (M + 255) / 256, policy, P, as_stream(stream), a, sk_ws, sk_bytes);
    HKP_LAUNCH_CHECK(who);
    return HKP_OK;
}

extern "C" int hkp_conv2d_fwd_x3(const hkp_conv_desc* d, const uint16_t* x_split, const uint16_t* w_split,
                                 const float* w_inv_scale, float* y, float* stat_partials, void* sk_workspace,
                                 int64_t sk_ws_bytes, hkp_stream_t stream) {
    HKP_CHECK_ARG(d && y, "hkp_conv2d_fwd_x3: null argument");
    return conv_fwd_x3_common(d, x_split, w_split, w_inv_scale, y, nullptr, stat_partials, sk_workspace, sk_ws_bytes,
                              3, stream, "hkp_conv2d_fwd_x3");
}

extern "C" int hkp_conv2d_fwd_x3_bnin(const hkp_conv_desc* d, const float* x_raw, const float* in_scale_shift,
                                      const uint16_t* w_split, const float* w_inv_scale, float* y, float* stat_partials,
                                      void* sk_workspace, int64_t sk_ws_bytes, hkp_stream_t stream) {
    HKP_CHECK_ARG(d && y && x_raw && in_scale_shift, "hkp_conv2d_fwd_x3_bnin: null argument");
    X3Args ep;
    ep.in_ss = in_scale_shift;
    return conv_fwd_x3_common(d, (const uint16_t*)x_raw, w_split, w_inv_scale, y, nullptr, stat_partials, sk_workspace,
                              sk_ws_bytes, 3, stream, "hkp_conv2d_fwd_x3_bnin", &ep);
}

extern "C" int hkp_conv2d_fwd_f16_bnin(const hkp_conv_desc* d, const uint16_t* x_raw_f16, const float* in_scale_shift,
                                       const uint16_t* w_f16, const float* w_inv_scale, uint16_t* y_f16,
                                       float* stat_partials, void* sk_workspace, int64_t sk_ws_bytes,
                                       hkp_stream_t stream) {
    HKP_CHECK_ARG(d && y_f16 && x_raw_f16 && in_scale_shift, "hkp_conv2d_fwd_f16_bnin: null argument");
    X3Args ep;
    ep.in_ss = in_scale_shift;
    return conv_fwd_x3_common(d, x_raw_f16, w_f16, w_inv_scale, nullptr, y_f16, stat_partials, sk_workspace,
                              sk_ws_bytes, 1, stream, "hkp_conv2d_fwd_f16_bnin", &ep);
}

extern "C" int hkp_conv2d_fwd_x3_products(const hkp_conv_desc* d, const uint16_t* x_split, const uint16_t* w_split,
                                          const float* w_inv_scale, int32_t products, float* y, float* stat_partials,
                                          void* sk_workspace, int64_t sk_ws_bytes, hkp_stream_t stream) {
    HKP_CHECK_ARG(d && y, "hkp_conv2d_fwd_x3_products: null argument");
    HKP_CHECK_ARG(products == HKP_X3_ALL || products == HKP_X3_W16 || products == HKP_X3_X16,
                  "hkp_conv2d_fwd_x3_products: unknown product set %d", products);
// ... 238 lines not shown

extern "C" int hkp_stem_pack_x3(const hkp_conv_desc* d, const float* x_nchw, uint16_t* x_split, hkp_stream_t stream) {
    return stem_pack(d, x_nchw, false, x_split, stream, "hkp_stem_pack_x3");
}

extern "C" int hkp_stem_pack_x3_u8(const hkp_conv_desc* d, const uint8_t* img_nhwc, uint16_t* x_split,
                                   hkp_stream_t stream) {
    return stem_pack(d, img_nhwc, true, x_split, stream, "hkp_stem_pack_x3_u8");
}

extern "C" int hkp_stem_weight_pack_x3(int32_t k, int32_t c, const float* w_oihw, uint16_t* w_split,
                                       float* w_inv_scale, hkp_stream_t stream) {
    HKP_CHECK_ARG(k > 0 && c >= 1 && c <= 4 && w_oihw && w_split && w_inv_scale, "hkp_stem_weight_pack_x3: bad args");
    hipLaunchKernelGGL(stem_weight_pack_x3_kernel, dim3(k), dim3(256), 0, as_stream(stream), c, w_oihw,
                       (_Float16*)w_split, w_inv_scale);
    HKP_LAUNCH_CHECK("hkp_stem_weight_pack_x3");
    return HKP_OK;
}

extern "C" int hkp_conv2d_fwd_stem_x3(const hkp_conv_desc* d, const uint16_t* x_split, const uint16_t* w_split,
                                      const float* w_inv_scale, float* y, float* stat_partials, hkp_stream_t stream) {
    int ho, wo;
    int rc = hkp_conv_out_hw(d, &ho, &wo);
    if (rc) return rc;
    HKP_CHECK_ARG(stem_x3_shape(d), "hkp_conv2d_fwd_stem_x3: needs the 7x7/s2/p3 NCHW stem with C<=4, Cout%%64==0");
    HKP_CHECK_ARG(x_split && w_split && y, "hkp_conv2d_fwd_stem_x3: null tensor");
    const long M = (long)d->n * ho * wo;
    HKP_CHECK_ARG(M < (1L << 31) && x3_offsets_fit(d->n, 2L * ho + 6, 2L * wo + 6, 8, d->k, 7),
                  "hkp_conv2d_fwd_stem_x3: too large");
    X3Args a;
    a.xs = (const _Float16*)x_split; a.ws = (const _Float16*)w_split; a.wscale = w_inv_scale;
    a.y = y; a.part = stat_partials; a.amax = nullptr; a.add = nullptr;
    a.N = d->n; a.H = 2 * ho + 6; a.W = 2 * wo + 6; a.C = 4; a.K = d->k; a.R = 7; a.S = 1;
    a.stride = 2; a.pad = 0; a.dil = 1; a.Ho = ho; a.Wo = wo;
    a.M = (int)M; a.cch = 1; a.RS = 7; a.nks = 7;
    a.plane = (long)d->n * a.H * a.W * 4;
    a.n_tiles = d->k / 64;
    a.stamps = g_x3_stamps;
    a.st_kind = g_x3_store;
    const long m_tiles = (M + 255) / 256;
    if (stem_patch_shape(ho, wo, d->k) && d->tile != HKP_TILE_64_PAIR) {
        hipLaunchKernelGGL(conv_x3_stem_patch_kernel<0>, dim3(m_tiles * a.n_tiles), dim3(512), 0, as_stream(stream), a);
        HKP_LAUNCH_CHECK("hkp_conv2d_fwd_stem_x3");
        return HKP_OK;
    }
    hipLaunchKernelGGL((conv_x3_kernel<64, true, true, 16, false, 3>), dim3(m_tiles * a.n_tiles), dim3(512), 0,
                       as_stream(stream), a);
    HKP_LAUNCH_CHECK("hkp_conv2d_fwd_stem_x3");
    return HKP_OK;
}

extern "C" int32_t hkp_stem_x3_image_ok(const hkp_conv_desc* d) {
    int ho, wo;
    if (!stem_x3_shape(d) || hkp_conv_out_hw(d, &ho, &wo) != HKP_OK) return 0;
    return stem_patch_shape(ho, wo, d->k) && d->tile != HKP_TILE_64_PAIR && (long)d->n * ho * wo < (1L << 31) ? 1 : 0;
}

extern "C" int hkp_conv2d_fwd_stem_x3_image(const hkp_conv_desc* d, const void* image, int32_t image_u8,
                                            const uint16_t* w_split, const float* w_inv_scale, float* y,
                                            float* stat_partials, hkp_stream_t stream) {
    HKP_CHECK_ARG(hkp_stem_x3_image_ok(d), "hkp_conv2d_fwd_stem_x3_image: shape not on the patch body "
                                           "(hkp_stem_x3_image_ok; use hkp_stem_pack_x3 + hkp_conv2d_fwd_stem_x3)");
    HKP_CHECK_ARG(image && w_split && y, "hkp_conv2d_fwd_stem_x3_image: null tensor");
    int ho, wo;
    hkp_conv_out_hw(d, &ho, &wo);
    X3Args a;
    a.xs = (const _Float16*)image; a.ws = (const _Float16*)w_split; a.wscale = w_inv_scale;
    a.y = y; a.part = stat_partials; a.amax = nullptr; a.add = nullptr;
    a.N = d->n; a.H = d->h; a.W = d->w; a.C = d->c; a.K = d->k; a.R = 7; a.S = 1;
    a.stride = 2; a.pad = 0; a.dil = 1; a.Ho = ho; a.Wo = wo;
    a.M = d->n * ho * wo; a.cch = 1; a.RS = 7; a.nks = 7; a.plane = 0;
    a.n_tiles = d->k / 64;
    a.stamps = g_x3_stamps;
    a.st_kind = g_x3_store;
    const dim3 grid((unsigned)(((long)a.M + 255) / 256 * a.n_tiles));
    if (image_u8) hipLaunchKernelGGL(conv_x3_stem_patch_kernel<2>, grid, dim3(512), 0, as_stream(stream), a);
    else hipLaunchKernelGGL(conv_x3_stem_patch_kernel<1>, grid, dim3(512), 0, as_stream(stream), a);
    HKP_LAUNCH_CHECK("hkp_conv2d_fwd_stem_x3_image");
    return HKP_OK;
}

extern "C" int32_t hkp_conv_x3_stat_tile_rows(const hkp_conv_desc* d, int32_t op) {
    HKP_CHECK_ARG(d, "hkp_conv_x3_stat_tile_rows: null descriptor");
    const bool packed = op == HKP_KOP_FWD_X3 || op == HKP_KOP_FWD_X3_W16 || op == HKP_KOP_FWD_X3_X16;
    if (packed && d->tile == HKP_TILE_192_A3 && d->k % 256 == 0) return 96;
    if (packed && d->tile == HKP_TILE_160_A3 && d->k % 128 == 0) return 80;
    return 128;
}

extern "C" int32_t hkp_conv_kernel_name(const hkp_conv_desc* d, int32_t op, int32_t stream_k_ok, char* buf,
                                        int32_t len) {
    HKP_CHECK_ARG(d && buf && len > 0, "hkp_conv_kernel_name: bad args");
    int ho, wo;
    int rc = hkp_conv_out_hw(d, &ho, &wo);
    if (rc) return rc;
    if (op != HKP_KOP_WGRAD_X3) {
        rc = check_tile(d, "hkp_conv_kernel_name");
        if (rc) return rc;
    }
    const bool sk = stream_k_ok != 0;
    switch (op) {
        case HKP_KOP_FWD_X3:
        case HKP_KOP_FWD_X3_W16:
        case HKP_KOP_FWD_X3_X16:
        case HKP_KOP_FWD_F16: {
            const int P = op == HKP_KOP_FWD_X3 ? 3 : op == HKP_KOP_FWD_X3_W16 ? 2 : op == HKP_KOP_FWD_X3_X16 ? 4 : 1;
            const long m = (long)d->n * ho * wo;
            const int cg = x3_packed(P) ? 32 : 64;
            const int nks = d->r * d->s * (d->c / cg);
            const bool halo = halo_shape(d->stride, d->r, d->s, d->pad, d->dilation, ho, wo, d->k) &&
                              (long)d->n * d->h * d->w * (d->c / cg * 64L) + 64 < (1L << 32);
            return x3_kernel_name(x3_choose(d->k, (m + 255) / 256, nks, sk, d->tile, x3_halo_level(halo, d->c / cg, P), P),
                                  false, P, buf, len);
        }
        case HKP_KOP_DGRAD_X3: {
            const long m = (long)d->n * d->h * d->w;
            const int nks = d->r * d->s * (d->k / 32);
            const int padp = d->dilation * (d->r - 1) - d->pad;
            const bool halo = halo_shape(d->stride, d->r, d->s, padp, d->dilation, d->h, d->w, d->c) &&
                              (long)d->n * ho * wo * (d->k / 32 * 64L) + 64 < (1L << 32);
            return x3_kernel_name(x3_choose(d->c, (m + 255) / 256, nks, sk, d->tile, x3_halo_level(halo, d->k / 32, 3), 3),
                                  false, 3, buf, len);
        }
        case HKP_KOP_STEM_X3:
            if (stem_patch_shape(ho, wo, d->k) && d->tile != HKP_TILE_64_PAIR)
                return snprintf(buf, len, "conv_x3_stem_patch_kernel<0>");
            return x3_kernel_name(X3_STEM, true, 3, buf, len);
        case HKP_KOP_STEM_X3_IMAGE:
        case HKP_KOP_STEM_X3_IMAGE_U8:
            HKP_CHECK_ARG(hkp_stem_x3_image_ok(d), "hkp_conv_kernel_name: the image stem needs the patch body's shape");
            return snprintf(buf, len, "conv_x3_stem_patch_kernel<%d>", op == HKP_KOP_STEM_X3_IMAGE ? 1 : 2);
        case HKP_KOP_WGRAD_X3: {
            HKP_CHECK_ARG(d->k % 64 == 0, "hkp_conv_kernel_name: wgrad needs Cout%%64==0");
            int sp, mps, ka, rt;
            wg_x3_plan(d, (long)d->n * ho * wo, wo, &sp, &mps, &ka, &rt);
            if (ka == 0) return snprintf(buf, len, "wgrad_x3_halo_kernel");
            return snprintf(buf, len, "wgrad_x3_kernel<%d>", ka);
        }
        default:
            HKP_CHECK_ARG(false, "hkp_conv_kernel_name: unknown op %d", op);
    }
    return HKP_ERR_BAD_ARG;
}

#ifdef HKP_AB_KNOBS
extern "C" void hkp_debug_x3_stamps(uint64_t* buf) { g_x3_stamps = (unsigned long long*)buf; }

extern "C" void hkp_debug_x3_stagger(int32_t ns) { g_x3_stagger_ns = ns > 0 ? ns : 0; }

extern "C" void hkp_debug_x3_split_tail(int32_t on) { g_x3_split_tail = on != 0; }
extern "C" void hkp_debug_stem_pair(int32_t on) { g_stem_pair = on != 0; }
extern "C" void hkp_debug_x3_pair128(int32_t on) { g_x3_pair128 = on != 0; }

extern "C" void hkp_debug_x3_store(int32_t kind) { g_x3_store = kind >= 0 && kind <= 4 ? kind : 0; }

extern "C" void hkp_debug_duo_stagger(int32_t ns) { g_duo_stagger_ns = ns; }

extern "C" void hkp_debug_x3_prio(int32_t mode) { g_x3_prio = mode >= 0 && mode <= 2 ? mode : 0; }

extern "C" void hkp_debug_x3_a_wrap(int32_t rows) { g_x3_a_wrap = rows > 0 ? rows : 0; }
#endif
```

### hulk-keypoints_amd/hkp/_lib.py

```python
import ctypes
import os

_HERE = os.path.dirname(os.path.abspath(__file__))
LIB_PATH = os.path.join(_HERE, "libhulkkp.so")

HKP_LAYOUT_NHWC = 0
HKP_LAYOUT_NCHW = 1
HKP_LOSS_BCE = 0
HKP_LOSS_MSE = 1


class HkpError(RuntimeError):
    pass


class ConvDesc(ctypes.Structure):
    _fields_ = [(n, ctypes.c_int32) for n in
                ("n", "h", "w", "c", "k", "r", "s", "stride", "pad", "dilation", "in_layout", "tile")]


(HKP_TILE_AUTO, HKP_TILE_NO_SK, HKP_TILE_SK, HKP_TILE_256, HKP_TILE_128_MF16, HKP_TILE_128_MF32, HKP_TILE_64_PAIR,
 HKP_TILE_RESERVED_7, HKP_TILE_RESERVED_8, HKP_TILE_256_TAIL, HKP_TILE_HALO, HKP_TILE_256_A3, HKP_TILE_AUTO_A3,
 HKP_TILE_DUO, HKP_TILE_RESERVED_14, HKP_TILE_192_A3, HKP_TILE_160_A3) = range(17)
HKP_KOP_FWD_X3, HKP_KOP_DGRAD_X3, HKP_KOP_FWD_F16, HKP_KOP_STEM_X3, HKP_KOP_WGRAD_X3, HKP_KOP_FWD_X3_W16, \
    HKP_KOP_FWD_X3_X16, HKP_KOP_STEM_X3_IMAGE, HKP_KOP_STEM_X3_IMAGE_U8 = range(9)
HKP_X3_W16, HKP_X3_ALL, HKP_X3_X16 = 2, 3, 4


class PackJob(ctypes.Structure):
    _fields_ = [("w", ctypes.c_void_p), ("out", ctypes.c_void_p), ("inv_scale", ctypes.c_void_p),
                ("kind", ctypes.c_int32), ("k", ctypes.c_int32), ("rs", ctypes.c_int32), ("c", ctypes.c_int32),
                ("r", ctypes.c_int32), ("s", ctypes.c_int32), ("pad", ctypes.c_int32), ("phase", ctypes.c_int32)]


class AdamTensor(ctypes.Structure):
    _fields_ = [("param", ctypes.c_void_p), ("grad", ctypes.c_void_p), ("exp_avg", ctypes.c_void_p),
                ("exp_avg_sq", ctypes.c_void_p), ("n", ctypes.c_int64)]


_P = ctypes.c_void_p
_I32 = ctypes.c_int32
_I64 = ctypes.c_int64
_F = ctypes.c_float
_CD = ctypes.POINTER(ConvDesc)

SIGNATURES = {
    "hkp_last_error": (ctypes.c_char_p, []),
    "hkp_version": (ctypes.c_char_p, []),
    "hkp_conv_out_hw": (ctypes.c_int, [_CD, ctypes.POINTER(_I32), ctypes.POINTER(_I32)]),
    "hkp_conv_stat_tiles": (_I64, [_CD]),
    "hkp_conv_x3_stat_tile_rows": (_I32, [_CD, _I32]),
    "hkp_conv2d_fwd": (ctypes.c_int, [_CD, _P, _P, _P, _P, _P]),
    "hkp_bn_finalize": (ctypes.c_int, [_I32, _I64, _I64, _I32, _P, _P, _P, _F, _F, _P, _P, _P, _P, _P, _P]),
    "hkp_bn_finalize_workspace_bytes": (_I64, [_I32, _I64]),
    "hkp_bn_finalize_ws": (ctypes.c_int, [_I32, _I64, _I64, _I32, _P, _P, _P, _F, _F, _P, _P, _P, _P, _P, _P, _I64,
                                          _P]),
    "hkp_bn_stats": (ctypes.c_int, [_I32, _I64, _I64, _I32, _P, _P, _P, _I64, _P]),
    "hkp_bn_finalize_ranks": (ctypes.c_int, [_I32, _I32, _P, _P, _P, _F, _F, _P, _P, _P, _P, _P, _P]),
    "hkp_bn_eval_params": (ctypes.c_int, [_I32, _P, _P, _P, _P, _F, _P, _P, _P]),
    "hkp_bn_apply": (ctypes.c_int, [_I64, _I32, _P, _P, _P, _P, _P, _I32, _P, _P, _I32, _P]),
    "hkp_bn_apply_f16": (ctypes.c_int, [_I64, _I32, _P, _P, _P, _P, _I32, _P, _P, _P]),
    "hkp_bn_relu_maxpool": (ctypes.c_int, [_I32, _I32, _I32, _I32, _P, _P, _P, _P, _I32, _P, _P]),
    "hkp_head_fc": (ctypes.c_int, [_I32, _I32, _I32, _I32, _P, _P, _P, _P, _P]),
    "hkp_bn_apply_head": (ctypes.c_int, [_I32, _I32, _I32, _I32, _I32, _P, _P, _P, _P, _I32, _P, _P, _P, _P]),
    "hkp_upsample_sigmoid": (ctypes.c_int, [_I32, _I32, _I32, _I32, _I32, _I32, _I32, _P, _P, _P, _P, _P]),
    "hkp_gauss_target": (ctypes.c_int, [_I32, _I32, _I32, _I32, _F, _P, _P, _P]),
    "hkp_weight_pack_x3": (ctypes.c_int, [_I32, _I32, _I32, _P, _P, _P, _P]),
    "hkp_conv2d_fwd_x3": (ctypes.c_int, [_CD, _P, _P, _P, _P, _P, _P, _I64, _P]),
    "hkp_conv2d_fwd_x3_products": (ctypes.c_int, [_CD, _P, _P, _P, _I32, _P, _P, _P, _I64, _P]),
    "hkp_conv2d_fwd_x3_bnin": (ctypes.c_int, [_CD, _P, _P, _P, _P, _P, _P, _P, _I64, _P]),
    "hkp_conv2d_fwd_f16_bnin": (ctypes.c_int, [_CD, _P, _P, _P, _P, _P, _P, _P, _I64, _P]),
    "hkp_conv_x3_sk_workspace_bytes": (_I64, []),
    "hkp_absmax": (ctypes.c_int, [_I64, _P, _P, _P]),
    "hkp_weight_pack_f16": (ctypes.c_int, [_I32, _I32, _P, _P, _P, _P]),
    "hkp_conv2d_fwd_f16": (ctypes.c_int, [_CD, _P, _P, _P, _P, _P, _P, _I64, _P]),
    "hkp_conv2d_fwd_f16_bn": (ctypes.c_int, [_CD, _P, _P, _P, _P, _P, _P, _I32, _P, _P, _I64, _P]),
    "hkp_gram_f16_workspace_bytes": (_I64, [_I64, _I32]),
    "hkp_gram_f16": (ctypes.c_int, [_I64, _I32, _P, _P, _P, _P, _I64, _P]),
    "hkp_bn_from_gram_workspace_bytes": (_I64, [_I32, _I32]),
    "hkp_bn_from_gram": (ctypes.c_int, [_I32, _I32, _I64, _P, _P, _P, _P, _P, _P, _F, _F, _P, _P, _P, _P, _P, _P,
                                        _I64, _P]),
    "hkp_conv_kernel_name": (_I32, [_CD, _I32, _I32, ctypes.c_char_p, _I32]),
    "hkp_upsample_argmax_ws_bytes": (_I64, [_I32, _I32, _I32, _I32]),
    "hkp_stem_pack_x3_elems": (_I64, [_CD]),
    "hkp_stem_pack_x3": (ctypes.c_int, [_CD, _P, _P, _P]),
    "hkp_stem_pack_x3_u8": (ctypes.c_int, [_CD, _P, _P, _P]),
    "hkp_images_u8_to_nchw": (ctypes.c_int, [_I32, _I32, _I32, _I32, _P, _P, _P]),
    "hkp_soft_argmax": (ctypes.c_int, [_I32, _I32, _I32, _I32, _F, _P, _P, _P]),
    "hkp_heat_overlay": (ctypes.c_int, [_I32, _I32, _I32, _I32, _P, _P, _P, _P, _P, _P]),
    "hkp_stem_weight_pack_x3": (ctypes.c_int, [_I32, _I32, _P, _P, _P, _P]),
    "hkp_conv2d_fwd_stem_x3": (ctypes.c_int, [_CD, _P, _P, _P, _P, _P, _P]),
    "hkp_stem_x3_image_ok": (_I32, [_CD]),
    "hkp_conv2d_fwd_stem_x3_image": (ctypes.c_int, [_CD, _P, _I32, _P, _P, _P, _P, _P]),
    "hkp_split_pack_x3": (ctypes.c_int, [_I64, _I32, _P, _P, _P, _P]),
    "hkp_weight_flip_pack_x3": (ctypes.c_int, [_CD, _P, _P, _P, _P]),
    "hkp_conv2d_bwd_data_x3": (ctypes.c_int, [_CD, _P, _P, _P, _P, _P, _P, _P, _I64, _P]),
    "hkp_phase_taps": (_I32, [_I32, _I32, _I32, _I32]),
    "hkp_conv2d_bwd_data_x3_strided": (ctypes.c_int, [_CD, _P, ctypes.POINTER(_P), ctypes.POINTER(_P), _P, _P, _P,
                                                       _P, _I64, _P]),
    "hkp_weight_pack_x3_batch_ws_bytes": (_I64, [_I32, ctypes.POINTER(PackJob)]),
    "hkp_weight_pack_x3_batch": (ctypes.c_int, [_I32, ctypes.POINTER(PackJob), _P, _I64, _P]),
    "hkp_conv_bwd_filter_x3_workspace": (_I64, [_CD]),
    "hkp_conv2d_bwd_filter_x3": (ctypes.c_int, [_CD, _P, _P, _P, _P, _P, _I64, _P]),
    "hkp_adam_step": (ctypes.c_int, [_I32, ctypes.POINTER(AdamTensor), _F, _F, _F, _F, _F, _F, _F, _P]),
    "hkp_conv_weight_flip":(ctypes.c_int, [_CD, _P, _P, _P]),
    "hkp_conv2d_bwd_data": (ctypes.c_int, [_CD, _P, _P, _P, _P, _P]),
    "hkp_conv_bwd_filter_workspace": (_I64, [_CD]),
    "hkp_conv2d_bwd_filter": (ctypes.c_int, [_CD, _P, _P, _P, _I32, _P, _I64, _P]),
    "hkp_bn_bwd_tiles": (_I64, [_I64]),
    "hkp_bn_bwd_reduce": (ctypes.c_int, [_I64, _I32, _P, _P, _P, _P, _P, _P, _P, _P, _P, _P]),
    "hkp_bn_bwd_finalize": (ctypes.c_int, [_I32, _I64, _P, _P, _P, _P, _P, _P, _P, _P, _P]),
    "hkp_bn_bwd_stats": (ctypes.c_int, [_I32, _I64, _P, _P, _P, _P, _P]),
    "hkp_bn_bwd_finalize_ranks": (ctypes.c_int, [_I32, _I32, _P, _P, _I32, _P, _P, _P, _P, _P, _P, _P]),
    "hkp_bn_bwd_apply": (ctypes.c_int, [_I64, _I32, _P, _P, _P, _P, _P, _P, _P, _P, _P, _P]),
    "hkp_maxpool_bwd": (ctypes.c_int, [_I32, _I32, _I32, _I32, _P, _P, _P, _P]),
    "hkp_heat_loss_workspace": (_I64, []),
    "hkp_heat_loss": (ctypes.c_int, [_I32, _I32, _I32, _I32, _I32, _P, _P, _P, _F, _P, _P, _P, _P]),
    "hkp_head_bwd_workspace": (_I64, [_I32, _I32, _I32, _I32]),
    "hkp_head_bwd": (ctypes.c_int, [_I32, _I32, _I32, _I32, _I32, _I32, _P, _P, _P, _P, _I64, _P]),
    "hkp_head_fc_bwd_workspace": (_I64, [_I32, _I32, _I32, _I32]),
    "hkp_head_fc_bwd": (ctypes.c_int, [_I32, _I32, _I32, _I32, _P, _P, _P, _P, _P, _P, _P, _I64, _P]),
    "hkp_jpeg_planes_bytes": (_I64, [_P]),
    "hkp_jpeg_reconstruct": (ctypes.c_int, [_I32, _P, _P, _P, _P, _I64, _P, _P]),
}

AB_SIGNATURES = {
    "hkp_debug_x3_stamps": (None, [_P]),
    "hkp_debug_x3_stagger": (None, [_I32]),
    "hkp_debug_x3_split_tail": (None, [_I32]),
    "hkp_debug_stem_pair": (None, [_I32]),
    "hkp_debug_fin_regs": (None, [_I32]),
    "hkp_debug_x3_pair128": (None, [_I32]),
    "hkp_debug_x3_store": (None, [_I32]),
    "hkp_debug_duo_stagger": (None, [_I32]),
    "hkp_debug_x3_prio": (None, [_I32]),
    "hkp_debug_x3_a_wrap": (None, [_I32]),
}
AB_LIB_PATH = os.path.join(os.path.dirname(os.path.dirname(_HERE)), "tools", "ab_lib", "libhulkkp_ab.so")

_lib = None
# ... 49 lines not shown
```

### hulk-keypoints_amd/hkp/ops.py

```python
import ctypes

import torch

from ._lib import (HKP_KOP_DGRAD_X3, HKP_KOP_FWD_F16, HKP_KOP_FWD_X3, HKP_KOP_FWD_X3_W16, HKP_KOP_FWD_X3_X16,
                   HKP_KOP_STEM_X3, HKP_KOP_STEM_X3_IMAGE, HKP_KOP_STEM_X3_IMAGE_U8, HKP_KOP_WGRAD_X3, HKP_X3_ALL,
                   HKP_LAYOUT_NCHW, HKP_LAYOUT_NHWC, HKP_TILE_160_A3, HKP_TILE_192_A3, ConvDesc, HkpError, call)

CONV_TILE_ROWS = 128

_observer = None


def set_observer(fn):
    global _observer
    _observer = fn


def conv_kernel_symbol(layout, cout):
    bn = 128 if cout % 128 == 0 else 64
    return "conv_fwd_kernel<128, %d, %s>" % (bn, "true" if layout != "nhwc" else "false")


def _stream():
    return ctypes.c_void_p(torch.cuda.current_stream().cuda_stream)


_sk_ws = {}


def _sk_workspace(enable=True):
    from ._lib import lib
    if not enable:
        return ctypes.c_void_p(0), ctypes.c_int64(0)
    st = torch.cuda.current_stream()
    key = (st.device_index, st.cuda_stream)
    ws = _sk_ws.get(key)
    if ws is None:
        nb = lib().hkp_conv_x3_sk_workspace_bytes()
        ws = torch.zeros(nb, device=torch.device("cuda", st.device_index), dtype=torch.uint8)
        _sk_ws[key] = ws
    return ctypes.c_void_p(ws.data_ptr()), ctypes.c_int64(ws.numel())


def _ptr(t):
    return ctypes.c_void_p(0 if t is None else t.data_ptr())


def _need(t, dtype, name, ndim=None):
    if not isinstance(t, torch.Tensor):
        raise HkpError("%s: expected a tensor" % name)
    if t.device.type != "cuda":
        raise HkpError("%s: tensor must be on the GPU (got %s)" % (name, t.device))
    if t.dtype != dtype:
        raise HkpError("%s: expected %s, got %s" % (name, dtype, t.dtype))
    if not t.is_contiguous():
        raise HkpError("%s: tensor must be contiguous" % name)
    if ndim is not None and t.dim() != ndim:
        raise HkpError("%s: expected %d dims, got %s" % (name, ndim, tuple(t.shape)))


def conv_out_hw(h, w, r, s, stride, pad, dil):
    return ((h + 2 * pad - dil * (r - 1) - 1) // stride + 1, (w + 2 * pad - dil * (s - 1) - 1) // stride + 1)


def conv2d_fwd(x, w, stride=1, pad=0, dil=1, layout="nhwc", stats=True, out=None):
    _need(x, torch.float32, "conv2d_fwd.x", 4)
    _need(w, torch.float32, "conv2d_fwd.w", 4)
    if layout == "nhwc":
        n, h, wd, c = x.shape
        k, r, s, cw = w.shape
        lay = HKP_LAYOUT_NHWC
    else:
        n, c, h, wd = x.shape
        k, cw, r, s = w.shape
        lay = HKP_LAYOUT_NCHW
    if cw != c:
        raise HkpError("conv2d_fwd: weight Cin %d != input C %d" % (cw, c))
    ho, wo = conv_out_hw(h, wd, r, s, stride, pad, dil)
    d = ConvDesc(n, h, wd, c, k, r, s, stride, pad, dil, lay)
    y = out if out is not None else torch.empty((n, ho, wo, k), device=x.device, dtype=torch.float32)
    _need(y, torch.float32, "conv2d_fwd.y", 4)
    if tuple(y.shape) != (n, ho, wo, k):
        raise HkpError("conv2d_fwd: out shape %s != %s" % (tuple(y.shape), (n, ho, wo, k)))
    part = None
    if stats:
        tiles = (n * ho * wo + CONV_TILE_ROWS - 1) // CONV_TILE_ROWS
        part = torch.empty((tiles, k, 2), device=x.device, dtype=torch.float32)
    def launch():
        call("hkp_conv2d_fwd", ctypes.byref(d), _ptr(x), _ptr(w), _ptr(y), _ptr(part), _stream())

    if _observer is None:
        launch()
    else:
        flops = 2.0 * n * ho * wo * k * r * s * c
        _observer(conv_kernel_symbol(layout, k), flops, 4.0 * (x.numel() + w.numel() + y.numel()), launch)
    return y, part


class PackedWeight(tuple):

    def __new__(cls, split, inv_scale):
        return super().__new__(cls, (split, inv_scale))

    @property
    def split(self):
        return self[0]

    @property
    def inv_scale(self):
        return self[1]


def kernel_name(d, op, sk=True):
    from ._lib import lib
    buf = ctypes.create_string_buffer(128)
    n = lib().hkp_conv_kernel_name(ctypes.byref(d), op, int(bool(sk)), buf, 128)
    if n < 0:
        raise HkpError("hkp_conv_kernel_name failed: %s" % lib().hkp_last_error().decode(errors="replace"))
    return buf.value.decode()


def weight_pack_x3(w):
    _need(w, torch.float32, "weight_pack_x3.w", 4)
    k, r, s, c = w.shape
    ws = torch.empty((k, r, s, 2 * c), device=w.device, dtype=torch.float16)
    sc = torch.empty(k, device=w.device, dtype=torch.float32)
    call("hkp_weight_pack_x3", k, r * s * c, c, _ptr(w), _ptr(ws), _ptr(sc), _stream())
    return PackedWeight(ws, sc)


def split_of(x):
    if x.dtype == torch.float16:
        return x, x._hkp_split_passes
    return getattr(x, "_hkp_split", None)


def channels_of(x):
    if x.dtype == torch.float16 and x._hkp_split_passes == 3:
        return x.shape[-1] // 2
    return x.shape[-1]


def _stat_partials(n_rows, k, device, part_out, name, tile_rows=CONV_TILE_ROWS):
    tiles = (n_rows + tile_rows - 1) // tile_rows
    if part_out is None:
        part = torch.empty((tiles, k, 2), device=device, dtype=torch.float32)
    else:
        _need(part_out, torch.float32, name, 3)
        if tuple(part_out.shape) != (tiles, k, 2):
            raise HkpError("%s: shape %s != %s" % (name, tuple(part_out.shape), (tiles, k, 2)))
        part = part_out
    if tile_rows != CONV_TILE_ROWS:
        part._hkp_tile_rows = tile_rows
    return part


def stat_tile_rows(part):
    return getattr(part, "_hkp_tile_rows", CONV_TILE_ROWS)


def conv2d_fwd_x3(xs, wp, stride=1, pad=0, dil=1, stats=True, out=None, part_out=None, sk=True, tile=0,
                  products=HKP_X3_ALL):
    ws, wsc = wp
    _need(xs, torch.float16, "conv2d_fwd_x3.x_split", 4)
    _need(ws, torch.float16, "conv2d_fwd_x3.w_split", 4)
    _need(wsc, torch.float32, "conv2d_fwd_x3.w_inv_scale", 1)
    n, h, wd, c2 = xs.shape
    k, r, s, cw2 = ws.shape
    if cw2 != c2:
        raise HkpError("conv2d_fwd_x3: weight Cin %d != input C %d" % (cw2 // 2, c2 // 2))
    c = c2 // 2
    ho, wo = conv_out_hw(h, wd, r, s, stride, pad, dil)
    d = ConvDesc(n, h, wd, c, k, r, s, stride, pad, dil, HKP_LAYOUT_NHWC, tile)
    y = out if out is not None else torch.empty((n, ho, wo, k), device=xs.device, dtype=torch.float32)
    kop = HKP_KOP_FWD_X3 if products == HKP_X3_ALL else HKP_KOP_FWD_X3_W16 if products == 2 else HKP_KOP_FWD_X3_X16
    part = None
    if stats:
        rows = CONV_TILE_ROWS
        if tile in (HKP_TILE_192_A3, HKP_TILE_160_A3):
            from ._lib import lib
            rows = lib().hkp_conv_x3_stat_tile_rows(ctypes.byref(d), kop)
        part = _stat_partials(n * ho * wo, k, xs.device, part_out, "conv2d_fwd_x3.part_out", rows)

    if products == HKP_X3_ALL:
        def launch():
            call("hkp_conv2d_fwd_x3", ctypes.byref(d), _ptr(xs), _ptr(ws), _ptr(wsc), _ptr(y), _ptr(part),
                 *_sk_workspace(sk), _stream())
    else:
        def launch():
            call("hkp_conv2d_fwd_x3_products", ctypes.byref(d), _ptr(xs), _ptr(ws), _ptr(wsc), int(products),
                 _ptr(y), _ptr(part), *_sk_workspace(sk), _stream())

    if _observer is None:
        launch()
    else:
        _observer(kernel_name(d, kop, sk), 2.0 * n * ho * wo * k * r * s * c,
                  2.0 * (xs.numel() + ws.numel()) + 4.0 * y.numel(), launch)
    return y, part


def bnin_kernel(n, h, w, c, k, r, s, stride, pad, dil, f16=False, tile=0, sk=True):
    cg = 64 if f16 else 32
    if c % cg or k % 64:
        return None
    try:
        ho, wo = conv_out_hw(h, w, r, s, stride, pad, dil)
    except HkpError:
        return None
    d = ConvDesc(n, h, w, c, k, r, s, stride, pad, dil, HKP_LAYOUT_NHWC, tile)
    name = kernel_name(d, HKP_KOP_FWD_F16 if f16 else HKP_KOP_FWD_X3, sk)
    if name.startswith("conv_x3_halo_kernel<"):
        return name.replace("_kernel<", "_bnin_kernel<")
    return None


def conv2d_fwd_bnin(y_in, in_ss, wp, stride=1, pad=1, dil=1, stats=True, sk=True, tile=0):
    ws, wsc = wp
    f16 = y_in.dtype == torch.float16
    _need(y_in, torch.float16 if f16 else torch.float32, "conv2d_fwd_bnin.y_in", 4)
    _need(in_ss, torch.float32, "conv2d_fwd_bnin.in_scale_shift", 1)
    _need(ws, torch.float16, "conv2d_fwd_bnin.w", 4)
    n, h, wd, c = y_in.shape
    k, r, s, cw = ws.shape
    if cw != (c if f16 else 2 * c):
        raise HkpError("conv2d_fwd_bnin: weight Cin %d != input C %d" % (cw if f16 else cw // 2, c))
    if in_ss.numel() != 2 * c:
        raise HkpError("conv2d_fwd_bnin: in_scale_shift size %d != 2C" % in_ss.numel())
    ho, wo = conv_out_hw(h, wd, r, s, stride, pad, dil)
    d = ConvDesc(n, h, wd, c, k, r, s, stride, pad, dil, HKP_LAYOUT_NHWC, tile)
    y = torch.empty((n, ho, wo, k), device=y_in.device, dtype=torch.float16 if f16 else torch.float32)
    part = _stat_partials(n * ho * wo, k, y_in.device, None, "conv2d_fwd_bnin") if stats else None
    fn = "hkp_conv2d_fwd_f16_bnin" if f16 else "hkp_conv2d_fwd_x3_bnin"

    def launch():
        call(fn, ctypes.byref(d), _ptr(y_in), _ptr(in_ss), _ptr(ws), _ptr(wsc), _ptr(y), _ptr(part),
             *_sk_workspace(sk), _stream())

    if _observer is None:
        launch()
    else:
        name = kernel_name(d, HKP_KOP_FWD_F16 if f16 else HKP_KOP_FWD_X3, sk).replace("_kernel<", "_bnin_kernel<")
        _observer(name, 2.0 * n * ho * wo * k * r * s * c,
                  y_in.element_size() * y_in.numel() + 2.0 * ws.numel() + y.element_size() * y.numel(), launch)
    return y, part


def weight_pack_f16(w):
    _need(w, torch.float32, "weight_pack_f16.w", 4)
    k, r, s, c = w.shape
    out = torch.empty((k, r, s, c), device=w.device, dtype=torch.float16)
    sc = torch.empty(k, device=w.device, dtype=torch.float32)
    call("hkp_weight_pack_f16", k, r * s * c, _ptr(w), _ptr(out), _ptr(sc), _stream())
    return PackedWeight(out, sc)


def conv2d_fwd_f16(x16, wp, stride=1, pad=0, dil=1, stats=True, sk=True, tile=0):
    ws, wsc = wp
    _need(x16, torch.float16, "conv2d_fwd_f16.x", 4)
    _need(ws, torch.float16, "conv2d_fwd_f16.w", 4)
    _need(wsc, torch.float32, "conv2d_fwd_f16.w_inv_scale", 1)
    n, h, wd, c = x16.shape
    k, r, s, cw = ws.shape
    if cw != c:
        raise HkpError("conv2d_fwd_f16: weight Cin %d != input C %d" % (cw, c))
    ho, wo = conv_out_hw(h, wd, r, s, stride, pad, dil)
# ... 119 lines not shown
    if u8:
        n, h, wd, c = x.shape
    else:
        n, c, h, wd = x.shape
    d = ConvDesc(n, h, wd, c, k, 7, 7, 2, 3, 1, HKP_LAYOUT_NCHW, tile)
    ho, wo = conv_out_hw(h, wd, 7, 7, 2, 3, 1)
    y = torch.empty((n, ho, wo, k), device=x.device, dtype=torch.float32)
    part = _stat_partials(n * ho * wo, k, x.device, part_out, "conv2d_fwd_stem_x3.part_out") if stats else None
    if image_direct is None:
        image_direct = STEM_IMAGE_DIRECT
    if image_direct and lib().hkp_stem_x3_image_ok(ctypes.byref(d)):
        xin = x.contiguous()
        op = HKP_KOP_STEM_X3_IMAGE_U8 if u8 else HKP_KOP_STEM_X3_IMAGE

        def launch():
            call("hkp_conv2d_fwd_stem_x3_image", ctypes.byref(d), _ptr(xin), 1 if u8 else 0, _ptr(ws), _ptr(wsc),
                 _ptr(y), _ptr(part), _stream())
        nbytes = float(xin.numel() * xin.element_size()) + 2.0 * ws.numel() + 4.0 * y.numel()
    else:
        xs = torch.empty(lib().hkp_stem_pack_x3_elems(ctypes.byref(d)), device=x.device, dtype=torch.float16)
        call("hkp_stem_pack_x3_u8" if u8 else "hkp_stem_pack_x3", ctypes.byref(d), _ptr(x), _ptr(xs), _stream())
        op = HKP_KOP_STEM_X3

        def launch():
            call("hkp_conv2d_fwd_stem_x3", ctypes.byref(d), _ptr(xs), _ptr(ws), _ptr(wsc), _ptr(y), _ptr(part),
                 _stream())
        nbytes = 2.0 * (xs.numel() + ws.numel()) + 4.0 * y.numel()
    if _observer is None:
        launch()
    else:
        _observer(kernel_name(d, op), 2.0 * n * ho * wo * k * 49 * c, nbytes, launch)
    return y, part


def images_u8_to_nchw(img):
    _need(img, torch.uint8, "images_u8_to_nchw.img", 4)
    n, h, w, c = img.shape
    x = torch.empty((n, c, h, w), device=img.device, dtype=torch.float32)
    call("hkp_images_u8_to_nchw", n, h, w, c, _ptr(img), _ptr(x), _stream())
    return x


def heat_overlay(heat, img, yx):
    _need(heat, torch.float32, "heat_overlay.heat", 4)
    _need(img, torch.uint8, "heat_overlay.img", 4)
    _need(yx, torch.int32, "heat_overlay.yx", 3)
    n, k, h, w = heat.shape
    if tuple(img.shape) != (n, h, w, 3) or tuple(yx.shape) != (n, k, 2):
        raise HkpError("heat_overlay: img %s / yx %s do not match heat %s" % (tuple(img.shape), tuple(yx.shape),
                                                                            tuple(heat.shape)))
    if k != 1 and k % 2:
        raise HkpError("heat_overlay: K must be 1 or even (two equal columns)")
    out = torch.empty((n, h, w, 3) if k == 1 else (n, h * (k // 2), 2 * w, 3), device=heat.device,
                      dtype=torch.uint8)
    mm = torch.empty(n * k * 2, device=heat.device, dtype=torch.float32)
    call("hkp_heat_overlay", n, k, h, w, _ptr(heat), _ptr(img), _ptr(yx), _ptr(mm), _ptr(out), _stream())
    return out


def soft_argmax(heat, beta=1.0):
    _need(heat, torch.float32, "soft_argmax.heat", 4)
    n, k, h, w = heat.shape
    out = torch.empty((n, k, 2), device=heat.device, dtype=torch.float32)
    call("hkp_soft_argmax", n, k, h, w, float(beta), _ptr(heat), _ptr(out), _stream())
    return out


FIN_TWO_LEVEL_TILES = 2048


def bn_finalize(part, count, gamma, beta, running_mean=None, running_var=None, num_batches_tracked=None,
                momentum=0.1, eps=1e-5, want_mean_invstd=True, two_level_tiles=FIN_TWO_LEVEL_TILES):
    _need(part, torch.float32, "bn_finalize.partials", 3)
    tiles, c, _ = part.shape
    ss = torch.empty(2 * c, device=part.device, dtype=torch.float32)
    mi = torch.empty(2 * c, device=part.device, dtype=torch.float32) if want_mean_invstd else None
    for t, nm in ((gamma, "gamma"), (beta, "beta"), (running_mean, "running_mean"), (running_var, "running_var")):
        if t is not None:
            _need(t, torch.float32, "bn_finalize." + nm, 1)
            if t.numel() != c:
                raise HkpError("bn_finalize.%s: %d != C=%d" % (nm, t.numel(), c))
    if num_batches_tracked is not None:
        _need(num_batches_tracked, torch.int64, "bn_finalize.num_batches_tracked")
    if tiles >= two_level_tiles:
        from ._lib import lib
        nb = lib().hkp_bn_finalize_workspace_bytes(c, tiles)
        ws = torch.empty((nb + 7) // 8, device=part.device, dtype=torch.float64)
        call("hkp_bn_finalize_ws", c, count, tiles, stat_tile_rows(part), _ptr(part), _ptr(gamma), _ptr(beta), momentum,
             eps, _ptr(running_mean), _ptr(running_var), _ptr(num_batches_tracked), _ptr(ss), _ptr(mi), _ptr(ws),
             nb, _stream())
        return ss, mi
    call("hkp_bn_finalize", c, count, tiles, stat_tile_rows(part), _ptr(part), _ptr(gamma), _ptr(beta), momentum, eps,
         _ptr(running_mean), _ptr(running_var), _ptr(num_batches_tracked), _ptr(ss), _ptr(mi), _stream())
    return ss, mi


def bn_stats(part, count, two_level_tiles=FIN_TWO_LEVEL_TILES):
    _need(part, torch.float32, "bn_stats.partials", 3)
    tiles, c, _ = part.shape
    st = torch.empty(2 * c + 1, device=part.device, dtype=torch.float64)
    ws, nb = None, 0
    if tiles >= two_level_tiles:
        from ._lib import lib
        nb = lib().hkp_bn_finalize_workspace_bytes(c, tiles)
        ws = torch.empty((nb + 7) // 8, device=part.device, dtype=torch.float64)
    call("hkp_bn_stats", c, count, tiles, stat_tile_rows(part), _ptr(part), _ptr(st), _ptr(ws), nb, _stream())
    return st


def bn_finalize_ranks(stats, gamma, beta, running_mean=None, running_var=None, num_batches_tracked=None,
                      momentum=0.1, eps=1e-5):
    _need(stats, torch.float64, "bn_finalize_ranks.stats", 2)
    r, l = stats.shape
    if l % 2 != 1:
        raise HkpError("bn_finalize_ranks.stats: row length %d is not 2C+1" % l)
    c = (l - 1) // 2
    for t, nm in ((gamma, "gamma"), (beta, "beta"), (running_mean, "running_mean"), (running_var, "running_var")):
        if t is not None:
            _need(t, torch.float32, "bn_finalize_ranks." + nm, 1)
            if t.numel() != c:
                raise HkpError("bn_finalize_ranks.%s: %d != C=%d" % (nm, t.numel(), c))
    if num_batches_tracked is not None:
        _need(num_batches_tracked, torch.int64, "bn_finalize_ranks.num_batches_tracked")
    ss = torch.empty(2 * c, device=stats.device, dtype=torch.float32)
    mi = torch.empty(2 * c, device=stats.device, dtype=torch.float32)
    call("hkp_bn_finalize_ranks", c, r, _ptr(stats.contiguous()), _ptr(gamma), _ptr(beta), momentum, eps,
         _ptr(running_mean), _ptr(running_var), _ptr(num_batches_tracked), _ptr(ss), _ptr(mi), _stream())
    return ss, mi


def bn_eval_params(gamma, beta, running_mean, running_var, eps=1e-5):
    c = running_mean.numel()
    ss = torch.empty(2 * c, device=running_mean.device, dtype=torch.float32)
    mi = torch.empty(2 * c, device=running_mean.device, dtype=torch.float32)
    call("hkp_bn_eval_params", c, _ptr(gamma), _ptr(beta), _ptr(running_mean), _ptr(running_var), eps, _ptr(ss),
         _ptr(mi), _stream())
    return ss, mi


def _split_out(shape, device, split):
    shp = tuple(shape[:-1]) + (shape[-1] * (2 if split == 3 else 1),)
    t = torch.empty(shp, device=device, dtype=torch.float16)
    t._hkp_split_passes = split
    return t


def _check_split(split, c, who):
    if split not in (0, 1, 3):
        raise HkpError("%s: split must be 0, 1 or 3" % who)
    if split and c % 32:
        raise HkpError("%s: split output needs C %% 32 == 0 (C=%d)" % (who, c))


def bn_apply(y, ss, res=None, res_ss=None, relu=True, out=None, split=0, keep_fp32=True):
    _need(y, torch.float32, "bn_apply.y")
    c = y.shape[-1]
    m = y.numel() // c
    _check_split(split, c, "bn_apply")
    if ss.numel() != 2 * c:
        raise HkpError("bn_apply: scale_shift size %d != 2C" % ss.numel())
    res_sp = None
    if res is not None and res.dtype == torch.float16:
        if res_ss is not None or getattr(res, "_hkp_split_passes", 0) != 3:
            raise HkpError("bn_apply: a split residual must be a packed (split=3) raw residual")
        _need(res, torch.float16, "bn_apply.res_split")
        if tuple(res.shape[:-1]) != tuple(y.shape[:-1]) or res.shape[-1] != 2 * c:
            raise HkpError("bn_apply: split residual shape %s vs %s" % (tuple(res.shape), tuple(y.shape)))
        res, res_sp = None, res
    elif res is not None:
        _need(res, torch.float32, "bn_apply.res")
        if res.shape != y.shape:
            raise HkpError("bn_apply: residual shape %s != %s" % (tuple(res.shape), tuple(y.shape)))
    if not keep_fp32 and not split:
        raise HkpError("bn_apply: keep_fp32=False needs a split output")
    o = None if not keep_fp32 else (out if out is not None else torch.empty_like(y))
    sp = _split_out(y.shape, y.device, split) if split else None
    call("hkp_bn_apply", m, c, _ptr(y), _ptr(ss), _ptr(res), _ptr(res_ss), _ptr(res_sp), int(bool(relu)), _ptr(o),
         _ptr(sp), int(split), _stream())
    if o is None:
        return sp
    if split:
        o._hkp_split = (sp, split)
    return o


def bn_apply_f16(y16, ss, res=None, res_ss=None, relu=True, keep_fp32=False):
    _need(y16, torch.float16, "bn_apply_f16.y")
    c = y16.shape[-1]
# ... 505 lines not shown
```

### include/hulkkp.h

```cpp
#ifndef HULKKP_H
#define HULKKP_H

#include <stddef.h>
#include <stdint.h>

#include "hkp_jpeg.h"

#ifdef __cplusplus
extern "C" {
#endif

#define HKP_OK 0
#define HKP_ERR_BAD_ARG (-1)
#define HKP_ERR_UNSUPPORTED (-2)

#define HKP_LAYOUT_NHWC 0
#define HKP_LAYOUT_NCHW 1

#define HKP_LOSS_BCE 0
#define HKP_LOSS_MSE 1

typedef void* hkp_stream_t;

const char* hkp_last_error(void);
const char* hkp_version(void);

typedef struct hkp_conv_desc {
    int32_t n, h, w, c;
    int32_t k, r, s;
    int32_t stride, pad, dilation;
    int32_t in_layout;
    int32_t tile;
} hkp_conv_desc;

#define HKP_TILE_AUTO 0
#define HKP_TILE_NO_SK 1
#define HKP_TILE_SK 2
#define HKP_TILE_256 3
#define HKP_TILE_128_MF16 4
#define HKP_TILE_128_MF32 5
#define HKP_TILE_64_PAIR 6
#define HKP_TILE_RESERVED_7 7
#define HKP_TILE_RESERVED_8 8
#define HKP_TILE_256_TAIL 9
#define HKP_TILE_HALO 10
#define HKP_TILE_AUTO_A3 12
#define HKP_TILE_256_A3 11
#define HKP_TILE_DUO 13
#define HKP_TILE_RESERVED_14 14
#define HKP_TILE_192_A3 15
#define HKP_TILE_160_A3 16

int hkp_conv_out_hw(const hkp_conv_desc* d, int32_t* ho, int32_t* wo);

int64_t hkp_conv_stat_tiles(const hkp_conv_desc* d);

int hkp_conv2d_fwd(const hkp_conv_desc* d, const float* x, const float* w, float* y,
                   float* stat_partials, hkp_stream_t stream);

int hkp_weight_pack_x3(int32_t k, int32_t rsc, int32_t c, const float* w, uint16_t* w_split, float* w_inv_scale,
                       hkp_stream_t stream);
int hkp_conv2d_fwd_x3(const hkp_conv_desc* d, const uint16_t* x_split, const uint16_t* w_split,
                      const float* w_inv_scale, float* y, float* stat_partials, void* sk_workspace,
                      int64_t sk_ws_bytes, hkp_stream_t stream);
int64_t hkp_conv_x3_sk_workspace_bytes(void);
#define HKP_X3_ALL 3
#define HKP_X3_W16 2
#define HKP_X3_X16 4
int hkp_conv2d_fwd_x3_products(const hkp_conv_desc* d, const uint16_t* x_split, const uint16_t* w_split,
                               const float* w_inv_scale, int32_t products, float* y, float* stat_partials,
                               void* sk_workspace, int64_t sk_ws_bytes, hkp_stream_t stream);
int hkp_conv2d_fwd_x3_bnin(const hkp_conv_desc* d, const float* x_raw, const float* in_scale_shift,
                           const uint16_t* w_split, const float* w_inv_scale, float* y, float* stat_partials,
                           void* sk_workspace, int64_t sk_ws_bytes, hkp_stream_t stream);
int hkp_conv2d_fwd_f16_bnin(const hkp_conv_desc* d, const uint16_t* x_raw_f16, const float* in_scale_shift,
                            const uint16_t* w_f16, const float* w_inv_scale, uint16_t* y_f16, float* stat_partials,
                            void* sk_workspace, int64_t sk_ws_bytes, hkp_stream_t stream);
int hkp_weight_pack_f16(int32_t k, int32_t rsc, const float* w, uint16_t* w_f16, float* w_inv_scale,
                        hkp_stream_t stream);
int hkp_conv2d_fwd_f16(const hkp_conv_desc* d, const uint16_t* x_f16, const uint16_t* w_f16,
                       const float* w_inv_scale, uint16_t* y_f16, float* stat_partials, void* sk_workspace,
                       int64_t sk_ws_bytes, hkp_stream_t stream);
int hkp_conv2d_fwd_f16_bn(const hkp_conv_desc* d, const uint16_t* x_f16, const uint16_t* w_f16,
                          const float* w_inv_scale, const float* scale_shift, const uint16_t* res_f16,
                          const float* res_scale_shift, int32_t relu, uint16_t* out_f16, void* sk_workspace,
                          int64_t sk_ws_bytes, hkp_stream_t stream);
int64_t hkp_gram_f16_workspace_bytes(int64_t m, int32_t c);
int hkp_gram_f16(int64_t m, int32_t c, const uint16_t* a, double* mean, double* second, void* workspace,
                 int64_t ws_bytes, hkp_stream_t stream);
int64_t hkp_bn_from_gram_workspace_bytes(int32_t k, int32_t c);
int hkp_bn_from_gram(int32_t k, int32_t c, int64_t count, const double* mean, const double* second,
                     const uint16_t* w_f16, const float* w_inv_scale, const float* gamma, const float* beta,
                     float momentum, float eps, float* running_mean, float* running_var,
                     int64_t* num_batches_tracked, float* scale_shift, float* mean_invstd, void* workspace,
                     int64_t ws_bytes, hkp_stream_t stream);
#define HKP_KOP_FWD_X3 0
#define HKP_KOP_DGRAD_X3 1
#define HKP_KOP_FWD_F16 2
#define HKP_KOP_STEM_X3 3
#define HKP_KOP_WGRAD_X3 4
#define HKP_KOP_FWD_X3_W16 5
#define HKP_KOP_FWD_X3_X16 6
#define HKP_KOP_STEM_X3_IMAGE 7
#define HKP_KOP_STEM_X3_IMAGE_U8 8
int32_t hkp_conv_kernel_name(const hkp_conv_desc* d, int32_t op, int32_t stream_k_ok, char* buf, int32_t len);
int32_t hkp_conv_x3_stat_tile_rows(const hkp_conv_desc* d, int32_t op);


int hkp_bn_finalize(int32_t c, int64_t count, int64_t tiles, int32_t tile_rows, const float* partials,
                    const float* gamma, const float* beta, float momentum, float eps,
                    float* running_mean, float* running_var, int64_t* num_batches_tracked,
                    float* scale_shift, float* mean_invstd, hkp_stream_t stream);

int64_t hkp_bn_finalize_workspace_bytes(int32_t c, int64_t tiles);
int hkp_bn_finalize_ws(int32_t c, int64_t count, int64_t tiles, int32_t tile_rows, const float* partials,
                       const float* gamma, const float* beta, float momentum, float eps,
                       float* running_mean, float* running_var, int64_t* num_batches_tracked,
                       float* scale_shift, float* mean_invstd, void* workspace, int64_t ws_bytes,
                       hkp_stream_t stream);

int hkp_bn_stats(int32_t c, int64_t count, int64_t tiles, int32_t tile_rows, const float* partials,
                 double* stats, void* workspace, int64_t ws_bytes, hkp_stream_t stream);
int hkp_bn_finalize_ranks(int32_t c, int32_t nranks, const double* stats, const float* gamma, const float* beta,
                          float momentum, float eps, float* running_mean, float* running_var,
                          int64_t* num_batches_tracked, float* scale_shift, float* mean_invstd,
                          hkp_stream_t stream);

int hkp_bn_eval_params(int32_t c, const float* gamma, const float* beta, const float* running_mean,
                       const float* running_var, float eps, float* scale_shift, float* mean_invstd,
                       hkp_stream_t stream);

int hkp_bn_apply(int64_t m, int32_t c, const float* y, const float* scale_shift, const float* res,
                 const float* res_scale_shift, const uint16_t* res_split, int32_t relu, float* out,
                 uint16_t* out_split, int32_t split_passes, hkp_stream_t stream);

int hkp_bn_apply_f16(int64_t m, int32_t c, const uint16_t* y, const float* scale_shift, const uint16_t* res,
                     const float* res_scale_shift, int32_t relu, uint16_t* out, float* out32, hkp_stream_t stream);

int hkp_bn_relu_maxpool(int32_t n, int32_t h, int32_t w, int32_t c, const float* y,
                        const float* scale_shift, float* out, uint16_t* out_split, int32_t split_passes,
                        uint8_t* route, hkp_stream_t stream);

int hkp_head_fc(int32_t n, int32_t hw, int32_t c, int32_t k, const float* feat, const float* w,
                const float* bias, float* lowres, hkp_stream_t stream);

int hkp_bn_apply_head(int32_t n, int32_t hw, int32_t c, int32_t k, int32_t y_f16, const void* y,
                      const float* scale_shift, const void* res, const float* res_scale_shift, int32_t res_kind,
                      const float* w, const float* bias, float* lowres, hkp_stream_t stream);

int64_t hkp_upsample_argmax_ws_bytes(int32_t n, int32_t k, int32_t H, int32_t W);
int hkp_upsample_sigmoid(int32_t n, int32_t k, int32_t h, int32_t w, int32_t H, int32_t W,
                         int32_t apply_sigmoid, const float* lowres, float* heat, uint64_t* argmax_ws, int32_t* argmax_yx,
                         hkp_stream_t stream);

int hkp_heat_overlay(int32_t n, int32_t k, int32_t H, int32_t W, const float* heat, const uint8_t* img_nhwc,
                     const int32_t* argmax_yx, float* minmax_ws, uint8_t* out, hkp_stream_t stream);

int hkp_soft_argmax(int32_t n, int32_t k, int32_t H, int32_t W, float beta, const float* heat, float* out_xy,
                    hkp_stream_t stream);

int hkp_gauss_target(int32_t n, int32_t k, int32_t H, int32_t W, float sigma, const float* uv,
                     double* out, hkp_stream_t stream);


int hkp_conv_weight_flip(const hkp_conv_desc* d, const float* w, float* w_flip, hkp_stream_t stream);

int hkp_conv2d_bwd_data(const hkp_conv_desc* d, const float* dy, const float* w_flip, const float* add, float* dx,
                        hkp_stream_t stream);

int hkp_absmax(int64_t n, const float* x, uint32_t* amax_bits, hkp_stream_t stream);

int64_t hkp_stem_pack_x3_elems(const hkp_conv_desc* d);
int hkp_stem_pack_x3(const hkp_conv_desc* d, const float* x_nchw, uint16_t* x_split, hkp_stream_t stream);
int hkp_stem_pack_x3_u8(const hkp_conv_desc* d, const uint8_t* img_nhwc, uint16_t* x_split, hkp_stream_t stream);
int hkp_images_u8_to_nchw(int32_t n, int32_t h, int32_t w, int32_t c, const uint8_t* img_nhwc, float* x_nchw,
                          hkp_stream_t stream);
int hkp_stem_weight_pack_x3(int32_t k, int32_t c, const float* w_oihw, uint16_t* w_split, float* w_inv_scale,
                            hkp_stream_t stream);
int hkp_conv2d_fwd_stem_x3(const hkp_conv_desc* d, const uint16_t* x_split, const uint16_t* w_split,
                           const float* w_inv_scale, float* y, float* stat_partials, hkp_stream_t stream);
int32_t hkp_stem_x3_image_ok(const hkp_conv_desc* d);
int hkp_conv2d_fwd_stem_x3_image(const hkp_conv_desc* d, const void* image, int32_t image_u8, const uint16_t* w_split,
                                 const float* w_inv_scale, float* y, float* stat_partials, hkp_stream_t stream);

int hkp_split_pack_x3(int64_t n, int32_t c, const float* x, const uint32_t* amax_bits, uint16_t* x_split,
                      hkp_stream_t stream);
int hkp_weight_flip_pack_x3(const hkp_conv_desc* d, const float* w, uint16_t* wf_split, float* wf_inv_scale,
                            hkp_stream_t stream);
int hkp_conv2d_bwd_data_x3(const hkp_conv_desc* d, const uint16_t* dy_split, const uint16_t* wf_split,
                           const float* wf_inv_scale, const uint32_t* dy_amax_bits, const float* add, float* dx,
                           void* sk_workspace, int64_t sk_ws_bytes, hkp_stream_t stream);
int32_t hkp_phase_taps(int32_t r, int32_t pad, int32_t stride, int32_t phase);
int hkp_conv2d_bwd_data_x3_strided(const hkp_conv_desc* d, const uint16_t* dy_split,
                                   const uint16_t* const* phase_split, const float* const* phase_inv_scale,
                                   const uint32_t* dy_amax_bits, const float* add, float* dx, void* sk_workspace,
                                   int64_t sk_ws_bytes, hkp_stream_t stream);
typedef struct hkp_pack_job {
    const float* w;
    uint16_t* out;
    float* inv_scale;
    int32_t kind, k, rs, c;
    int32_t r, s, pad, phase;
// ... 66 lines not shown
```

Measured before the change: 1873 images/sec.

## Add mixed-tile-size A3 conv schedule with segmented BN stat partials

Adds a new HKP_TILE_MIX_A3 tile mode that splits the conv M dimension into up to three segments of different tile heights, aiming to reduce wave-quantization tail across CUs. BN finalize and stats kernels gain a segmented layout so per-tile partial rows can vary by segment, and the Python side propagates the segment table from the conv stat layout. This adds per-tile segment lookups in the finalize kernels. Whether the new mode runs depends on the tile selector choosing MIX_A3.

```diff
diff --git a/hulk-keypoints_amd/csrc/bn.hip b/hulk-keypoints_amd/csrc/bn.hip
--- a/hulk-keypoints_amd/csrc/bn.hip
+++ b/hulk-keypoints_amd/csrc/bn.hip
@@ -12,12 +12,39 @@
     if (c == 0) stats[2 * C] = (double)count;
 }
 
-template <int CPB, int NT = 256, int NB = 0>
+struct FinSegs {
+    int n = 1;
+    int rows[3] = {0, 0, 0};
+    long t0[3] = {0, 0, 0};
+    long r0[3] = {0, 0, 0};
+    long tiles = 0;
+};
+template <bool SEG>
+__device__ __forceinline__ long fin_tile_rows(long t, int tile_rows, long count, const FinSegs& g, int& full) {
+    if constexpr (!SEG) {
+        full = tile_rows;
+        return min((long)tile_rows, count - t * tile_rows);
+    } else {
+        const bool s2 = g.n > 2 && t >= g.t0[2], s1 = g.n > 1 && t >= g.t0[1];
+        full = s2 ? g.rows[2] : s1 ? g.rows[1] : g.rows[0];
+        const long tb = s2 ? g.t0[2] : s1 ? g.t0[1] : 0, rb = s2 ? g.r0[2] : s1 ? g.r0[1] : 0;
+        return min((long)full, count - (rb + (t - tb) * full));
+    }
+}
+__device__ __forceinline__ long fin_seg_row0(long t, long count, const FinSegs& g) {
+    if (t >= g.tiles) return count;
+    const bool s2 = g.n > 2 && t >= g.t0[2], s1 = g.n > 1 && t >= g.t0[1];
+    const long full = s2 ? g.rows[2] : s1 ? g.rows[1] : g.rows[0];
+    const long tb = s2 ? g.t0[2] : s1 ? g.t0[1] : 0, rb = s2 ? g.r0[2] : s1 ? g.r0[1] : 0;
+    return rb + (t - tb) * full;
+}
+
+template <int CPB, int NT = 256, int NB = 0, bool SEG = false>
 __global__ __launch_bounds__(NT) void bn_finalize_kernel(int C, long count, long tiles, int tile_rows,
                                                          const float* __restrict__ part, const float* gamma,
                                                          const float* beta, float momentum, float eps, float* rmean,
                                                          float* rvar, int64_t* nbt, float* ss, float* mi,
-                                                         double* stats) {
+                                                         double* stats, FinSegs sg) {
     constexpr int TL = NT / CPB, NW = NT / 64;
     __shared__ double red[NW][8];
     const int cl = threadIdx.x % CPB, tl = threadIdx.x / CPB, c = blockIdx.x * CPB + cl;
@@ -33,15 +60,18 @@
 #pragma unroll
         for (int j = 0; j < NB; ++j) s += (double)v[j].x;
         const double mean = lanes_sum_d<CPB, NW>(s, red) / (double)count;
-        const bool pow2 = (tile_rows & (tile_rows - 1)) == 0;
-        const double inv_rows = 1.0 / (double)tile_rows;
+        const int rows0 = SEG ? sg.rows[0] : tile_rows;
+        const bool pow2 = (rows0 & (rows0 - 1)) == 0;
+        const double inv_rows = 1.0 / (double)rows0;
         double q = 0.0;
 #pragma unroll
         for (int j = 0; j < NB; ++j) {
             const long t = tl + (long)j * TL;
             if (ok && t < tiles) {
-                const long n_t = min((long)tile_rows, count - t * tile_rows);
-                const double tm = pow2 && n_t == tile_rows ? (double)v[j].x * inv_rows : (double)v[j].x / (double)n_t;
+                int full;
+                const long n_t = fin_tile_rows<SEG>(t, tile_rows, count, sg, full);
+                const bool fast = pow2 && n_t == rows0 && (!SEG || sg.n == 1 || t < sg.t0[1]);
+                const double tm = fast ? (double)v[j].x * inv_rows : (double)v[j].x / (double)n_t;
                 const double dm = tm - mean;
                 q += (double)v[j].y + (double)n_t * dm * dm;
             }
@@ -79,7 +109,8 @@
             for (int j = 0; j < 8; ++j) {
                 const long t = t0 + (long)j * TL;
                 if (t < tiles) {
-                    const long n_t = min((long)tile_rows, count - t * tile_rows);
+                    int full;
+                    const long n_t = fin_tile_rows<SEG>(t, tile_rows, count, sg, full);
                     const double dm = (double)v[j].x / (double)n_t - mean;
                     q += (double)v[j].y + (double)n_t * dm * dm;
                 }
@@ -108,8 +139,10 @@
     return a[0];
 }
 
+template <bool SEG = false>
 __global__ __launch_bounds__(1024) void bn_fin_chunk_kernel(int C, long count, long tiles, int tile_rows,
-                                                            const float* __restrict__ part, double2* __restrict__ ws) {
+                                                            const float* __restrict__ part, double2* __restrict__ ws,
+                                                            FinSegs sg) {
     __shared__ double red[FIN_TL][64];
     const int cl = threadIdx.x & 63, tl = threadIdx.x >> 6, c = blockIdx.x * 64 + cl;
     const bool ok = c < C;
@@ -125,14 +158,16 @@
     for (int j = 0; j < FIN_TPL; ++j) s += (double)v[j].x;
     const double S = fin_col_sum(s, red, tl, cl);
     const long te = min(tiles, t0 + FIN_CHUNK);
-    const long nk = min(count, te * (long)tile_rows) - t0 * (long)tile_rows;
+    const long nk = SEG ? fin_seg_row0(te, count, sg) - fin_seg_row0(t0, count, sg)
+                        : min(count, te * (long)tile_rows) - t0 * (long)tile_rows;
     const double mk = S / (double)nk;
     double q = 0.0;
 #pragma unroll
     for (int j = 0; j < FIN_TPL; ++j) {
         const long t = t0 + tl + (long)FIN_TL * j;
         if (t < tiles) {
-            const long n_t = min((long)tile_rows, count - t * tile_rows);
+            int full;
+            const long n_t = fin_tile_rows<SEG>(t, tile_rows, count, sg, full);
             const double dm = (double)v[j].x / (double)n_t - mk;
             q += (double)v[j].y + (double)n_t * dm * dm;
         }
@@ -141,11 +176,12 @@
     if (tl == 0 && ok) ws[blockIdx.y * (long)C + c] = make_double2(S, Q);
 }
 
+template <bool SEG = false>
 __global__ __launch_bounds__(1024) void bn_fin_merge_kernel(int C, long count, long chunks, int tile_rows,
                                                             const double2* __restrict__ ws, const float* gamma,
                                                             const float* beta, float momentum, float eps,
                                                             float* rmean, float* rvar, int64_t* nbt, float* ss,
-                                                            float* mi, double* stats) {
+                                                            float* mi, double* stats, FinSegs sg) {
     __shared__ double red[FIN_TL][64];
     const int cl = threadIdx.x & 63, tl = threadIdx.x >> 6, c = blockIdx.x * 64 + cl;
     const bool ok = c < C;
@@ -158,7 +194,8 @@
     if (ok)
         for (long k = tl; k < chunks; k += FIN_TL) {
             const double2 w = ws[k * C + c];
-            const long nk = min(rows, count - k * rows);
+            const long nk = SEG ? fin_seg_row0((k + 1) * FIN_CHUNK, count, sg) - fin_seg_row0(k * FIN_CHUNK, count, sg)
+                                : min(rows, count - k * rows);
             const double dm = w.x / (double)nk - mean;
             q += w.y + (double)nk * dm * dm;
         }
@@ -408,18 +445,22 @@
 static int fin_one(const char* who, int32_t c, int64_t count, int64_t tiles, int32_t tile_rows, const float* partials,
                    const float* gamma, const float* beta, float momentum, float eps, float* running_mean,
                    float* running_var, int64_t* num_batches_tracked, float* scale_shift, float* mean_invstd,
-                   double* stats, hkp_stream_t stream) {
+                   double* stats, hkp_stream_t stream, const FinSegs* segs = nullptr) {
     HKP_CHECK_ARG(c > 0 && count > 0 && tiles > 0 && tile_rows > 0, "%s: bad sizes", who);
     HKP_CHECK_ARG(partials && (scale_shift || stats), "%s: null tensor", who);
     HKP_CHECK_ARG((running_mean == nullptr) == (running_var == nullptr), "%s: running stats pair", who);
-    HKP_CHECK_ARG((tiles - 1) * (int64_t)tile_rows < count && tiles * (int64_t)tile_rows >= count,
+    HKP_CHECK_ARG(segs || ((tiles - 1) * (int64_t)tile_rows < count && tiles * (int64_t)tile_rows >= count),
                   "%s: tiles/tile_rows inconsistent with count", who);
+    const FinSegs sg = segs ? *segs : FinSegs{};
     const int cpb = partials_cpb(c);
     const long per = g_fin_regs ? (tiles + 256 / cpb - 1) / (256 / cpb) : 1L << 40;
-#define HKP_FIN1(CPB, NT, NB)                                                                                      \
-    hipLaunchKernelGGL((bn_finalize_kernel<CPB, NT, NB>), dim3((c + CPB - 1) / CPB), dim3(NT), 0, as_stream(stream), \
-                       c, (long)count, (long)tiles, tile_rows, partials, gamma, beta, momentum, eps, running_mean,   \
-                       running_var, num_batches_tracked, scale_shift, mean_invstd, stats)
+#define HKP_FIN2(CPB, NT, NB, SEG)                                                                                \
+    hipLaunchKernelGGL((bn_finalize_kernel<CPB, NT, NB, SEG>), dim3((c + CPB - 1) / CPB), dim3(NT), 0,             \
+                       as_stream(stream), c, (long)count, (long)tiles, tile_rows, partials, gamma, beta, momentum, \
+                       eps, running_mean, running_var, num_batches_tracked, scale_shift, mean_invstd, stats, sg)
+#define HKP_FIN1(CPB, NT, NB)                    \
+    if (segs) { HKP_FIN2(CPB, NT, NB, true); } \
+    else { HKP_FIN2(CPB, NT, NB, false); }
 #define HKP_FIN(CPB)                                  \
     if (tiles >= 4096) { HKP_FIN1(CPB, 1024, 0); } \
     else if (per <= 8) { HKP_FIN1(CPB, 256, 8); } \
@@ -432,6 +473,7 @@
     else { HKP_FIN(1); }
 #undef HKP_FIN
 #undef HKP_FIN1
+#undef HKP_FIN2
     HKP_LAUNCH_CHECK(who);
     return HKP_OK;
 }
@@ -444,24 +486,59 @@
 static int fin_two(const char* who, int32_t c, int64_t count, int64_t tiles, int32_t tile_rows, const float* partials,
                    const float* gamma, const float* beta, float momentum, float eps, float* running_mean,
                    float* running_var, int64_t* num_batches_tracked, float* scale_shift, float* mean_invstd,
-                   double* stats, void* workspace, int64_t ws_bytes, hkp_stream_t stream) {
+                   double* stats, void* workspace, int64_t ws_bytes, hkp_stream_t stream,
+                   const FinSegs* segs = nullptr) {
     HKP_CHECK_ARG(c > 0 && count > 0 && tiles > 0 && tile_rows > 0, "%s: bad sizes", who);
     HKP_CHECK_ARG(partials && (scale_shift || stats) && workspace, "%s: null tensor", who);
     HKP_CHECK_ARG((running_mean == nullptr) == (running_var == nullptr), "%s: running stats pair", who);
-    HKP_CHECK_ARG((tiles - 1) * (int64_t)tile_rows < count && tiles * (int64_t)tile_rows >= count,
+    HKP_CHECK_ARG(segs || ((tiles - 1) * (int64_t)tile_rows < count && tiles * (int64_t)tile_rows >= count),
                   "%s: tiles/tile_rows inconsistent with count", who);
+    const FinSegs sg = segs ? *segs : FinSegs{};
     const int64_t need = hkp_bn_finalize_workspace_bytes(c, tiles);
     HKP_CHECK_ARG(ws_bytes >= need, "%s: workspace %ld < %ld", who, (long)ws_bytes, (long)need);
     const long chunks = (tiles + FIN_CHUNK - 1) / FIN_CHUNK;
     hipStream_t st = as_stream(stream);
     const unsigned cg = (unsigned)((c + 63) / 64);
-    hipLaunchKernelGGL(bn_fin_chunk_kernel, dim3(cg, (unsigned)chunks), dim3(1024), 0, st, c, (long)count,
-                       (long)tiles, tile_rows, partials, (double2*)workspace);
+    if (segs)
+        hipLaunchKernelGGL(bn_fin_chunk_kernel<true>, dim3(cg, (unsigned)chunks), dim3(1024), 0, st, c, (long)count,
+                           (long)tiles, tile_rows, partials, (double2*)workspace, sg);
+    else
+        hipLaunchKernelGGL(bn_fin_chunk_kernel<false>, dim3(cg, (unsigned)chunks), dim3(1024), 0, st, c, (long)count,
+                           (long)tiles, tile_rows, partials, (double2*)workspace, sg);
     HKP_LAUNCH_CHECK(who);
-    hipLaunchKernelGGL(bn_fin_merge_kernel, dim3(cg), dim3(1024), 0, st, c, (long)count, chunks, tile_rows,
-                       (const double2*)workspace, gamma, beta, momentum, eps, running_mean, running_var,
-                       num_batches_tracked, scale_shift, mean_invstd, stats);
+    if (segs)
+        hipLaunchKernelGGL(bn_fin_merge_kernel<true>, dim3(cg), dim3(1024), 0, st, c, (long)count, chunks, tile_rows,
+                           (const double2*)workspace, gamma, beta, momentum, eps, running_mean, running_var,
+                           num_batches_tracked, scale_shift, mean_invstd, stats, sg);
+    else
+        hipLaunchKernelGGL(bn_fin_merge_kernel<false>, dim3(cg), dim3(1024), 0, st, c, (long)count, chunks, tile_rows,
+                           (const double2*)workspace, gamma, beta, momentum, eps, running_mean, running_var,
+                           num_batches_tracked, scale_shift, mean_invstd, stats, sg);
     HKP_LAUNCH_CHECK(who);
+    return HKP_OK;
+}
+
+static int fin_segs(const char* who, int64_t count, int32_t nseg, const int32_t* segments, FinSegs* sg, int64_t* tiles) {
+    HKP_CHECK_ARG(segments && nseg >= 1 && nseg <= 3 && count > 0, "%s: 1 to 3 segments", who);
+    int64_t row = 0, t = 0;
+    sg->n = nseg;
+    for (int i = 0; i < nseg; ++i) {
+        const int64_t rows = segments[2 * i], nt = segments[2 * i + 1];
+        HKP_CHECK_ARG(rows > 0 && nt > 0, "%s: segment %d: bad rows/tiles", who, i);
+        sg->rows[i] = (int)rows;
+        sg->t0[i] = t;
+        sg->r0[i] = row;
+        if (i + 1 < nseg) {
+            row += rows * nt;
+            HKP_CHECK_ARG(row < count, "%s: segment %d reaches past count", who, i);
+        } else {
+            HKP_CHECK_ARG(row + (nt - 1) * rows < count && row + nt * rows >= count,
+                          "%s: segments inconsistent with count", who);
+        }
+        t += nt;
+    }
+    sg->tiles = t;
+    *tiles = t;
     return HKP_OK;
 }
 
@@ -493,6 +570,40 @@
                        nullptr, nullptr, nullptr, nullptr, stats, workspace, ws_bytes, stream);
     return fin_one("hkp_bn_stats", c, count, tiles, tile_rows, partials, nullptr, nullptr, 0.f, 0.f, nullptr, nullptr,
                    nullptr, nullptr, nullptr, stats, stream);
+}
+
+extern "C" int hkp_bn_finalize_seg(int32_t c, int64_t count, int32_t nseg, const int32_t* segments,
+                                   const float* partials, const float* gamma, const float* beta, float momentum,
+                                   float eps, float* running_mean, float* running_var, int64_t* num_batches_tracked,
+                                   float* scale_shift, float* mean_invstd, void* workspace, int64_t ws_bytes,
+                                   hkp_stream_t stream) {
+    HKP_CHECK_ARG(scale_shift, "hkp_bn_finalize_seg: null tensor");
+    FinSegs sg;
+    int64_t tiles = 0;
+    const int rc = fin_segs("hkp_bn_finalize_seg", count, nseg, segments, &sg, &tiles);
+    if (rc) return rc;
+    const FinSegs* ps = nseg > 1 ? &sg : nullptr;
+    if (workspace)
+        return fin_two("hkp_bn_finalize_seg", c, count, tiles, sg.rows[0], partials, gamma, beta, momentum, eps,
+                       running_mean, running_var, num_batches_tracked, scale_shift, mean_invstd, nullptr, workspace,
+                       ws_bytes, stream, ps);
+    return fin_one("hkp_bn_finalize_seg", c, count, tiles, sg.rows[0], partials, gamma, beta, momentum, eps,
+                   running_mean, running_var, num_batches_tracked, scale_shift, mean_invstd, nullptr, stream, ps);
+}
+
+extern "C" int hkp_bn_stats_seg(int32_t c, int64_t count, int32_t nseg, const int32_t* segments, const float* partials,
+                                double* stats, void* workspace, int64_t ws_bytes, hkp_stream_t stream) {
+    HKP_CHECK_ARG(stats, "hkp_bn_stats_seg: null tensor");
+    FinSegs sg;
+    int64_t tiles = 0;
+    const int rc = fin_segs("hkp_bn_stats_seg", count, nseg, segments, &sg, &tiles);
+    if (rc) return rc;
+    const FinSegs* ps = nseg > 1 ? &sg : nullptr;
+    if (workspace)
+        return fin_two("hkp_bn_stats_seg", c, count, tiles, sg.rows[0], partials, nullptr, nullptr, 0.f, 0.f, nullptr,
+                       nullptr, nullptr, nullptr, nullptr, stats, workspace, ws_bytes, stream, ps);
+    return fin_one("hkp_bn_stats_seg", c, count, tiles, sg.rows[0], partials, nullptr, nullptr, 0.f, 0.f, nullptr,
+                   nullptr, nullptr, nullptr, nullptr, stats, stream, ps);
 }
 
 extern "C" int hkp_bn_finalize_ranks(int32_t c, int32_t nranks, const double* stats, const float* gamma,
diff --git a/hulk-keypoints_amd/csrc/conv_x3.hip b/hulk-keypoints_amd/csrc/conv_x3.hip
--- a/hulk-keypoints_amd/csrc/conv_x3.hip
+++ b/hulk-keypoints_amd/csrc/conv_x3.hip
@@ -27,6 +27,8 @@
     long plane;
     int ost = 0, OH = 0, OW = 0, oy = 0, ox = 0;
     int mt0 = 0;
+    int m_base = 0, part_base = 0;
+    int mix_b1 = 0, mix_b2 = 0, mix_m1 = 0, mix_m2 = 0, mix_p1 = 0, mix_p2 = 0;
     long sk_units = 0;
     float* sk_ws = nullptr;
     unsigned* sk_cnt = nullptr;
@@ -258,7 +260,7 @@
         for (int j = 0; j < NJ; ++j) red[wm * BN + wn * NJ * CW + j * CW + lane] = colsum[j];
     }
     __syncthreads();
-    const long tile128 = (long)(m0 >> 7);
+    const long tile128 = (long)a.part_base + ((m0 - a.m_base) >> 7);
     for (int e = tid; e < 2 * BN; e += 512) {
         const int h = e / BN, c = e - h * BN;
         const int cnt = min(128, a.M - (m0 + 128 * h));
@@ -359,7 +361,7 @@
                 }
                 x3_chan_merge(S[0], Q[0], S[1], Q[1], 1.f / (16 * NI), 8.f * NI);
                 const float sc = wide[32 * BN + c];
-                const long tile128 = (long)(m0 / (2 * WROWS)) + h;
+                const long tile128 = (long)a.part_base + (m0 - a.m_base) / (2 * WROWS) + h;
                 a.part[(tile128 * a.K + n0 + c) * 2 + 0] = S[0] * sc;
                 a.part[(tile128 * a.K + n0 + c) * 2 + 1] = Q[0] * (sc * sc);
             }
@@ -432,7 +434,7 @@
     }
     if constexpr (WMP == 2) {
         if (nw == 0 || lane >= CW) return;
-        const long pt = (long)(m0 / WROWS) + wm;
+        const long pt = (long)a.part_base + (m0 - a.m_base) / WROWS + wm;
 #pragma unroll
         for (int j = 0; j < NJ; ++j) {
             const int c = wn * NJ * CW + j * CW + lane;
@@ -453,7 +455,7 @@
     lds_sync();
     const int nb = min(WROWS, max(0, a.M - (m0 + WROWS * (wm | 1))));
     if ((wm & 1) || nw == 0 || lane >= CW) return;
-    const long tile128 = (long)(m0 / (2 * WROWS)) + (wm >> 1);
+    const long tile128 = (long)a.part_base + (m0 - a.m_base) / (2 * WROWS) + (wm >> 1);
     const float ia = 1.f / (float)nw, ib = nb > 0 ? 1.f / (float)nb : 0.f;
     const float f = (float)nw * (float)nb / (float)(nw + nb);
 #pragma unroll
@@ -905,7 +907,7 @@
     static_assert(!A_SINK || A3, "the A sink is the A3 body's");
 
     const int mt = tile / a.n_tiles, nt = tile - mt * a.n_tiles;
-    const int m0 = (mt + a.mt0) * BM, n0 = nt * BN;
+    const int m0 = a.m_base + (mt + a.mt0) * BM, n0 = nt * BN;
     const int tid = threadIdx.x, lane = tid & 63;
     const int w = __builtin_amdgcn_readfirstlane(tid >> 6);
     const int wm = w / WN, wn = w % WN;
@@ -1266,6 +1268,30 @@
     __shared__ __attribute__((aligned(1024))) char smem[x3_a3_lds(160, 128)];
     x3_stamp(a, 0);
     conv_x3_tile<128, false, false, 16, P, true, 160>(a, smem, xcd_remap(blockIdx.x, gridDim.x), 0, a.nks, false);
+}
+
+template <int P>
+__global__ __launch_bounds__(512, 1) void conv_x3_a3_mix_kernel(X3Args a) {
+    __shared__ __attribute__((aligned(1024))) char smem[X3_A3_LDS];
+    x3_stagger(a);
+    x3_stamp(a, 0);
+    const int b = blockIdx.x;
+    if (b < a.mix_b1) {
+        conv_x3_tile<256, false, false, 16, P, true, 256>(a, smem, xcd_remap(b, a.mix_b1), 0, a.nks, false);
+        return;
+    }
+    X3Args t = a;
+    if (b < a.mix_b2) {
+        t.m_base = a.mix_m1;
+        t.part_base = a.mix_p1;
+        conv_x3_tile<256, false, false, 16, P, true, 192>(t, smem, xcd_remap(b - a.mix_b1, a.mix_b2 - a.mix_b1), 0,
+                                                          a.nks, false);
+        return;
+    }
+    t.m_base = a.mix_m2;
+    t.part_base = a.mix_p2;
+    conv_x3_tile<256, false, false, 16, P, true, 160>(t, smem, xcd_remap(b - a.mix_b2, (int)gridDim.x - a.mix_b2), 0,
+                                                      a.nks, false);
 }
 
 template <int BN, int P>
@@ -2898,7 +2924,52 @@
     bool a3 = false;
     bool duo = false;
     int bm = 256;
+    bool mix = false;
 };
+
+struct X3Mix {
+    int cost = 0;
+    int rounds[3] = {0, 0, 0};
+    long mt[3] = {0, 0, 0};
+    long m_base[3] = {0, 0, 0};
+    long part_base[3] = {0, 0, 0};
+    long part_tiles = 0;
+};
+static constexpr int X3_MIX_BM[3] = {256, 192, 160};
+static X3Mix x3_mix_plan(long M, int n_tiles, int G) {
+    X3Mix p;
+    if (M <= 0 || n_tiles <= 0 || G / n_tiles <= 0) return p;
+    const long R = G / n_tiles, need = (M + R - 1) / R;
+    const long a_hi = (need + 255) / 256, a_lo = std::max<long>(0, (need - 3 * 192 - 7 * 160) / 256);
+    long best = -1, ba = 0, bb = 0, bc = 0;
+    for (long a = a_hi; a >= a_lo; --a)
+        for (long b = 3; b >= 0; --b)
+            for (long c = 0; c <= 7; ++c) {
+                if (256 * a + 192 * b + 160 * c < need) continue;
+                const long cost = 16 * a + 12 * b + 10 * c;
+                if (best < 0 || cost < best) { best = cost; ba = a; bb = b; bc = c; }
+                break;
+            }
+    if (best < 0 || best > (1L << 30)) return p;
+    p.cost = (int)best;
+    p.rounds[0] = (int)ba; p.rounds[1] = (int)bb; p.rounds[2] = (int)bc;
+    const int last = bc ? 2 : bb ? 1 : 0;
+    long row = 0, pt = 0;
+    for (int r = 0; r < 3; ++r) {
+        const long bm = X3_MIX_BM[r], left = M - row;
+        p.m_base[r] = row;
+        p.part_base[r] = pt;
+        p.mt[r] = r == last ? (left + bm - 1) / bm : p.rounds[r] * R;
+        const long rows = r == last ? left : p.mt[r] * bm;
+        row += rows;
+        pt += (rows + bm / 2 - 1) / (bm / 2);
+    }
+    p.part_tiles = pt;
+    return p;
+}
+static bool x3_mix_ok(int k, long m_tiles, int P) {
+    return x3_packed(P) && k % 256 == 0 && m_tiles * (k / 256) > x3_cus();
+}
 static X3Choice x3_choose_base(int k, long m_tiles, int nks, bool sk_ok, int policy, int halo);
 static X3Choice x3_choose(int k, long m_tiles, int nks, bool sk_ok, int policy, int halo, int P);
 HKP_AB_KNOB(int, g_x3_pair128, 1);
@@ -2914,6 +2985,7 @@
     if (policy == HKP_TILE_256_A3 && P == 3 && k % 256 != 0 && g_x3_pair128) policy = HKP_TILE_AUTO;
     if (policy == HKP_TILE_192_A3 && (!x3_packed(P) || k % 256 != 0)) policy = HKP_TILE_AUTO;
     if (policy == HKP_TILE_160_A3 && (!x3_packed(P) || k % 128 != 0)) policy = HKP_TILE_AUTO;
+    if (policy == HKP_TILE_MIX_A3 && !x3_mix_ok(k, m_tiles, P)) policy = HKP_TILE_AUTO;
     if (policy != HKP_TILE_AUTO_A3 && policy != HKP_TILE_AUTO) return x3_choose_base(k, m_tiles, nks, sk_ok, policy, halo);
     X3Choice c = x3_choose_base(k, m_tiles, nks, sk_ok, HKP_TILE_AUTO, halo);
     if (c.bn == 256 && !c.sk && !c.halo && !c.pair) c.a3 = true;
@@ -2932,7 +3004,7 @@
 static X3Choice x3_choose_base(int k, long m_tiles, int nks, bool sk_ok, int policy, int halo) {
     if ((halo >= 1 && policy == HKP_TILE_HALO) ||
         (halo == 2 && (policy == HKP_TILE_AUTO || policy == HKP_TILE_256_TAIL || policy == HKP_TILE_256_A3 ||
-                       policy == HKP_TILE_192_A3 || policy == HKP_TILE_160_A3))) {
+                       policy == HKP_TILE_192_A3 || policy == HKP_TILE_160_A3 || policy == HKP_TILE_MIX_A3))) {
         X3Choice c{64, 16, true, false};
         c.halo = true;
         return c;
@@ -2963,6 +3035,11 @@
                 return c;
             }
             break;
+        case HKP_TILE_MIX_A3: {
+            X3Choice c{256, 16, false, false, false, true};
+            c.mix = true;
+            return c;
+        }
         default:
             break;
     }
@@ -2979,6 +3056,7 @@
 static int x3_kernel_name(const X3Choice& c, bool stem, int P, char* buf, int len) {
     if (c.halo) return snprintf(buf, len, "conv_x3_halo_kernel<%d>", P);
     if (c.duo) return snprintf(buf, len, "conv_x3_duo_kernel<%d>", P);
+    if (c.mix) return snprintf(buf, len, "conv_x3_a3_mix_kernel<%d>", P);
     if (c.a3)
         return snprintf(buf, len, c.bm == 192                  ? "conv_x3_a3_192_kernel<%d>"
                                   : c.bm == 160 && c.bn == 128 ? "conv_x3_a3_160x128_kernel<%d>"
@@ -3070,6 +3148,20 @@
         } else {
             x3_dispatch_p(P, [&](auto pc) { hipLaunchKernelGGL(conv_x3_halo_kernel<pc.value>, gh, dim3(512), 0, st, a); });
         }
+        return;
+    }
+    if (c.mix) {
+        const X3Mix mp = x3_mix_plan(a.M, a.n_tiles, x3_cus());
+        X3Args t = a;
+        t.mix_b1 = (int)(mp.mt[0] * a.n_tiles);
+        t.mix_b2 = (int)((mp.mt[0] + mp.mt[1]) * a.n_tiles);
+        t.mix_m1 = (int)mp.m_base[1]; t.mix_m2 = (int)mp.m_base[2];
+        t.mix_p1 = (int)mp.part_base[1]; t.mix_p2 = (int)mp.part_base[2];
+        const dim3 gx((unsigned)((mp.mt[0] + mp.mt[1] + mp.mt[2]) * a.n_tiles));
+        x3_dispatch_p(P, [&](auto pc) {
+            if constexpr (x3_packed(pc.value))
+                hipLaunchKernelGGL(conv_x3_a3_mix_kernel<pc.value>, gx, dim3(512), 0, st, t);
+        });
         return;
     }
     if (c.bm != 256) {
@@ -3165,7 +3257,7 @@
 }
 
 static int check_tile(const hkp_conv_desc* d, const char* who) {
-    HKP_CHECK_ARG(d->tile >= HKP_TILE_AUTO && d->tile <= HKP_TILE_160_A3, "%s: unknown tile policy %d", who,
+    HKP_CHECK_ARG(d->tile >= HKP_TILE_AUTO && d->tile <= HKP_TILE_MIX_A3, "%s: unknown tile policy %d", who,
                   d->tile);
     HKP_CHECK_ARG(d->tile != HKP_TILE_RESERVED_7 && d->tile != HKP_TILE_RESERVED_8 && d->tile != HKP_TILE_RESERVED_14,
                   "%s: tile policy %d is retired (a persistent conv body, measured slower)", who, d->tile);
@@ -3570,10 +3662,70 @@
 
 extern "C" int32_t hkp_conv_x3_stat_tile_rows(const hkp_conv_desc* d, int32_t op) {
     HKP_CHECK_ARG(d, "hkp_conv_x3_stat_tile_rows: null descriptor");
-    const bool packed = op == HKP_KOP_FWD_X3 || op == HKP_KOP_FWD_X3_W16 || op == HKP_KOP_FWD_X3_X16;
-    if (packed && d->tile == HKP_TILE_192_A3 && d->k % 256 == 0) return 96;
-    if (packed && d->tile == HKP_TILE_160_A3 && d->k % 128 == 0) return 80;
-    return 128;
+    if (op != HKP_KOP_FWD_X3 && op != HKP_KOP_FWD_X3_W16 && op != HKP_KOP_FWD_X3_X16 && op != HKP_KOP_FWD_F16) return 128;
+    int32_t seg[6];
+    const int n = hkp_conv_x3_stat_layout(d, op, seg);
+    return n < 0 ? n : seg[0];
+}
+
+static int x3_fwd_choice(const hkp_conv_desc* d, int32_t op, bool sk, X3Choice* c, long* m_out, const char* who) {
+    int ho, wo;
+    int rc = hkp_conv_out_hw(d, &ho, &wo);
+    if (rc) return rc;
+    rc = check_tile(d, who);
+    if (rc) return rc;
+    HKP_CHECK_ARG(op == HKP_KOP_FWD_X3 || op == HKP_KOP_FWD_X3_W16 || op == HKP_KOP_FWD_X3_X16 || op == HKP_KOP_FWD_F16,
+                  "%s: not a forward conv op %d", who, op);
+    const int P = op == HKP_KOP_FWD_X3 ? 3 : op == HKP_KOP_FWD_X3_W16 ? 2 : op == HKP_KOP_FWD_X3_X16 ? 4 : 1;
+    const long m = (long)d->n * ho * wo;
+    const int cg = x3_packed(P) ? 32 : 64;
+    const int nks = d->r * d->s * (d->c / cg);
+    const bool halo = halo_shape(d->stride, d->r, d->s, d->pad, d->dilation, ho, wo, d->k) &&
+                      (long)d->n * d->h * d->w * (d->c / cg * 64L) + 64 < (1L << 32);
+    *c = x3_choose(d->k, (m + 255) / 256, nks, sk, d->tile, x3_halo_level(halo, d->c / cg, P), P);
+    *m_out = m;
+    return HKP_OK;
+}
+
+extern "C" int32_t hkp_conv_x3_stat_layout(const hkp_conv_desc* d, int32_t op, int32_t* segments) {
+    HKP_CHECK_ARG(d && segments, "hkp_conv_x3_stat_layout: null argument");
+    X3Choice c{64, 16, true, false};
+    long m = 0;
+    const int rc = x3_fwd_choice(d, op, true, &c, &m, "hkp_conv_x3_stat_layout");
+    if (rc) return rc < 0 ? rc : -rc;
+    for (int i = 0; i < 6; ++i) segments[i] = 0;
+    if (c.mix) {
+        const X3Mix mp = x3_mix_plan(m, d->k / 256, x3_cus());
+        int n = 0;
+        for (int r = 0; r < 3; ++r) {
+            if (mp.mt[r] == 0) continue;
+            const long end = r == 2 ? mp.part_tiles : mp.part_base[r + 1];
+            segments[2 * n] = X3_MIX_BM[r] / 2;
+            segments[2 * n + 1] = (int32_t)(end - mp.part_base[r]);
+            ++n;
+        }
+        return n;
+    }
+    const int rows = c.halo || c.duo || c.bm == 256 ? 128 : c.bm / 2;
+    segments[0] = rows;
+    segments[1] = (int32_t)((m + rows - 1) / rows);
+    return 1;
+}
+
+extern "C" int32_t hkp_conv_x3_mix_plan(int64_t m, int32_t n_tiles, int32_t cus, int32_t* out) {
+    HKP_CHECK_ARG(out && m > 0 && m < (1L << 31) && n_tiles > 0 && cus > 0, "hkp_conv_x3_mix_plan: bad args");
+    const X3Mix mp = x3_mix_plan(m, n_tiles, cus);
+    out[0] = mp.cost;
+    int n = 0;
+    for (int r = 0; r < 3; ++r) {
+        out[1 + r] = mp.rounds[r];
+        out[4 + r] = (int32_t)mp.mt[r];
+        out[7 + r] = (int32_t)mp.m_base[r];
+        out[10 + r] = (int32_t)mp.part_base[r];
+        n += mp.mt[r] > 0;
+    }
+    out[13] = (int32_t)mp.part_tiles;
+    return n;
 }
 
 extern "C" int32_t hkp_conv_kernel_name(const hkp_conv_desc* d, int32_t op, int32_t stream_k_ok, char* buf,
diff --git a/hulk-keypoints_amd/hkp/_lib.py b/hulk-keypoints_amd/hkp/_lib.py
--- a/hulk-keypoints_amd/hkp/_lib.py
+++ b/hulk-keypoints_amd/hkp/_lib.py
@@ -21,10 +21,11 @@
 
 (HKP_TILE_AUTO, HKP_TILE_NO_SK, HKP_TILE_SK, HKP_TILE_256, HKP_TILE_128_MF16, HKP_TILE_128_MF32, HKP_TILE_64_PAIR,
  HKP_TILE_RESERVED_7, HKP_TILE_RESERVED_8, HKP_TILE_256_TAIL, HKP_TILE_HALO, HKP_TILE_256_A3, HKP_TILE_AUTO_A3,
- HKP_TILE_DUO, HKP_TILE_RESERVED_14, HKP_TILE_192_A3, HKP_TILE_160_A3) = range(17)
+ HKP_TILE_DUO, HKP_TILE_RESERVED_14, HKP_TILE_192_A3, HKP_TILE_160_A3, HKP_TILE_MIX_A3) = range(18)
 HKP_KOP_FWD_X3, HKP_KOP_DGRAD_X3, HKP_KOP_FWD_F16, HKP_KOP_STEM_X3, HKP_KOP_WGRAD_X3, HKP_KOP_FWD_X3_W16, \
     HKP_KOP_FWD_X3_X16, HKP_KOP_STEM_X3_IMAGE, HKP_KOP_STEM_X3_IMAGE_U8 = range(9)
 HKP_X3_W16, HKP_X3_ALL, HKP_X3_X16 = 2, 3, 4
+HKP_MIX_PLAN_LEN = 14
 
 
 class PackJob(ctypes.Structure):
@@ -50,12 +51,17 @@
     "hkp_conv_out_hw": (ctypes.c_int, [_CD, ctypes.POINTER(_I32), ctypes.POINTER(_I32)]),
     "hkp_conv_stat_tiles": (_I64, [_CD]),
     "hkp_conv_x3_stat_tile_rows": (_I32, [_CD, _I32]),
+    "hkp_conv_x3_stat_layout": (_I32, [_CD, _I32, ctypes.POINTER(_I32)]),
+    "hkp_conv_x3_mix_plan": (_I32, [_I64, _I32, _I32, ctypes.POINTER(_I32)]),
     "hkp_conv2d_fwd": (ctypes.c_int, [_CD, _P, _P, _P, _P, _P]),
     "hkp_bn_finalize": (ctypes.c_int, [_I32, _I64, _I64, _I32, _P, _P, _P, _F, _F, _P, _P, _P, _P, _P, _P]),
     "hkp_bn_finalize_workspace_bytes": (_I64, [_I32, _I64]),
     "hkp_bn_finalize_ws": (ctypes.c_int, [_I32, _I64, _I64, _I32, _P, _P, _P, _F, _F, _P, _P, _P, _P, _P, _P, _I64,
                                           _P]),
     "hkp_bn_stats": (ctypes.c_int, [_I32, _I64, _I64, _I32, _P, _P, _P, _I64, _P]),
+    "hkp_bn_finalize_seg": (ctypes.c_int, [_I32, _I64, _I32, ctypes.POINTER(_I32), _P, _P, _P, _F, _F, _P, _P, _P, _P,
+                                           _P, _P, _I64, _P]),
+    "hkp_bn_stats_seg": (ctypes.c_int, [_I32, _I64, _I32, ctypes.POINTER(_I32), _P, _P, _P, _I64, _P]),
     "hkp_bn_finalize_ranks": (ctypes.c_int, [_I32, _I32, _P, _P, _P, _F, _F, _P, _P, _P, _P, _P, _P]),
     "hkp_bn_eval_params": (ctypes.c_int, [_I32, _P, _P, _P, _P, _F, _P, _P, _P]),
     "hkp_bn_apply": (ctypes.c_int, [_I64, _I32, _P, _P, _P, _P, _P, _I32, _P, _P, _I32, _P]),
diff --git a/hulk-keypoints_amd/hkp/ops.py b/hulk-keypoints_amd/hkp/ops.py
--- a/hulk-keypoints_amd/hkp/ops.py
+++ b/hulk-keypoints_amd/hkp/ops.py
@@ -4,7 +4,7 @@
 
 from ._lib import (HKP_KOP_DGRAD_X3, HKP_KOP_FWD_F16, HKP_KOP_FWD_X3, HKP_KOP_FWD_X3_W16, HKP_KOP_FWD_X3_X16,
                    HKP_KOP_STEM_X3, HKP_KOP_STEM_X3_IMAGE, HKP_KOP_STEM_X3_IMAGE_U8, HKP_KOP_WGRAD_X3, HKP_X3_ALL,
-                   HKP_LAYOUT_NCHW, HKP_LAYOUT_NHWC, HKP_TILE_160_A3, HKP_TILE_192_A3, ConvDesc, HkpError, call)
+                   HKP_LAYOUT_NCHW, HKP_LAYOUT_NHWC, HKP_TILE_160_A3, HKP_TILE_192_A3, HKP_TILE_MIX_A3, ConvDesc, HkpError, call)
 
 CONV_TILE_ROWS = 128
 
@@ -141,8 +141,12 @@
     return x.shape[-1]
 
 
-def _stat_partials(n_rows, k, device, part_out, name, tile_rows=CONV_TILE_ROWS):
+def _stat_partials(n_rows, k, device, part_out, name, tile_rows=CONV_TILE_ROWS, segments=None):
     tiles = (n_rows + tile_rows - 1) // tile_rows
+    if segments is not None and len(segments) > 1:
+        tiles = sum(t for _, t in segments)
+    else:
+        segments = None
     if part_out is None:
         part = torch.empty((tiles, k, 2), device=device, dtype=torch.float32)
     else:
@@ -152,11 +156,32 @@
         part = part_out
     if tile_rows != CONV_TILE_ROWS:
         part._hkp_tile_rows = tile_rows
+    if segments is not None:
+        part._hkp_segments = tuple(segments)
     return part
 
 
 def stat_tile_rows(part):
     return getattr(part, "_hkp_tile_rows", CONV_TILE_ROWS)
+
+
+def stat_segments(part):
+    return getattr(part, "_hkp_segments", None)
+
+
+def conv_stat_layout(d, kop):
+    from ._lib import lib
+    seg = (ctypes.c_int32 * 6)()
+    n = lib().hkp_conv_x3_stat_layout(ctypes.byref(d), kop, seg)
+    if n < 1:
+        raise HkpError("hkp_conv_x3_stat_layout failed (rc=%d): %s"
+                       % (n, lib().hkp_last_error().decode(errors="replace")))
+    return tuple((seg[2 * i], seg[2 * i + 1]) for i in range(n))
+
+
+def _seg_table(segments):
+    flat = [v for rt in segments for v in rt]
+    return (ctypes.c_int32 * len(flat))(*flat)
 
 
 def conv2d_fwd_x3(xs, wp, stride=1, pad=0, dil=1, stats=True, out=None, part_out=None, sk=True, tile=0,
@@ -176,11 +201,11 @@
     kop = HKP_KOP_FWD_X3 if products == HKP_X3_ALL else HKP_KOP_FWD_X3_W16 if products == 2 else HKP_KOP_FWD_X3_X16
     part = None
     if stats:
-        rows = CONV_TILE_ROWS
-        if tile in (HKP_TILE_192_A3, HKP_TILE_160_A3):
-            from ._lib import lib
-            rows = lib().hkp_conv_x3_stat_tile_rows(ctypes.byref(d), kop)
-        part = _stat_partials(n * ho * wo, k, xs.device, part_out, "conv2d_fwd_x3.part_out", rows)
+        rows, segs = CONV_TILE_ROWS, None
+        if tile in (HKP_TILE_192_A3, HKP_TILE_160_A3, HKP_TILE_MIX_A3):
+            segs = conv_stat_layout(d, kop)
+            rows = segs[0][0]
+        part = _stat_partials(n * ho * wo, k, xs.device, part_out, "conv2d_fwd_x3.part_out", rows, segs)
 
     if products == HKP_X3_ALL:
         def launch():
@@ -466,6 +491,17 @@
                 raise HkpError("bn_finalize.%s: %d != C=%d" % (nm, t.numel(), c))
     if num_batches_tracked is not None:
         _need(num_batches_tracked, torch.int64, "bn_finalize.num_batches_tracked")
+    segs = stat_segments(part)
+    if segs is not None:
+        ws, nb = None, 0
+        if tiles >= two_level_tiles:
+            from ._lib import lib
+            nb = lib().hkp_bn_finalize_workspace_bytes(c, tiles)
+            ws = torch.empty((nb + 7) // 8, device=part.device, dtype=torch.float64)
+        call("hkp_bn_finalize_seg", c, count, len(segs), _seg_table(segs), _ptr(part), _ptr(gamma), _ptr(beta),
+             momentum, eps, _ptr(running_mean), _ptr(running_var), _ptr(num_batches_tracked), _ptr(ss), _ptr(mi),
+             _ptr(ws), nb, _stream())
+        return ss, mi
     if tiles >= two_level_tiles:
         from ._lib import lib
         nb = lib().hkp_bn_finalize_workspace_bytes(c, tiles)
@@ -488,6 +524,10 @@
         from ._lib import lib
         nb = lib().hkp_bn_finalize_workspace_bytes(c, tiles)
         ws = torch.empty((nb + 7) // 8, device=part.device, dtype=torch.float64)
+    segs = stat_segments(part)
+    if segs is not None:
+        call("hkp_bn_stats_seg", c, count, len(segs), _seg_table(segs), _ptr(part), _ptr(st), _ptr(ws), nb, _stream())
+        return st
     call("hkp_bn_stats", c, count, tiles, stat_tile_rows(part), _ptr(part), _ptr(st), _ptr(ws), nb, _stream())
     return st
 
diff --git a/include/hulkkp.h b/include/hulkkp.h
--- a/include/hulkkp.h
+++ b/include/hulkkp.h
@@ -50,6 +50,7 @@
 #define HKP_TILE_RESERVED_14 14
 #define HKP_TILE_192_A3 15
 #define HKP_TILE_160_A3 16
+#define HKP_TILE_MIX_A3 17
 
 int hkp_conv_out_hw(const hkp_conv_desc* d, int32_t* ho, int32_t* wo);
 
@@ -105,6 +106,9 @@
 #define HKP_KOP_STEM_X3_IMAGE_U8 8
 int32_t hkp_conv_kernel_name(const hkp_conv_desc* d, int32_t op, int32_t stream_k_ok, char* buf, int32_t len);
 int32_t hkp_conv_x3_stat_tile_rows(const hkp_conv_desc* d, int32_t op);
+int32_t hkp_conv_x3_stat_layout(const hkp_conv_desc* d, int32_t op, int32_t* segments);
+#define HKP_MIX_PLAN_LEN 14
+int32_t hkp_conv_x3_mix_plan(int64_t m, int32_t n_tiles, int32_t cus, int32_t* out);
 
 
 int hkp_bn_finalize(int32_t c, int64_t count, int64_t tiles, int32_t tile_rows, const float* partials,
@@ -118,6 +122,14 @@
                        float* running_mean, float* running_var, int64_t* num_batches_tracked,
                        float* scale_shift, float* mean_invstd, void* workspace, int64_t ws_bytes,
                        hkp_stream_t stream);
+
+int hkp_bn_finalize_seg(int32_t c, int64_t count, int32_t nseg, const int32_t* segments, const float* partials,
+                        const float* gamma, const float* beta, float momentum, float eps,
+                        float* running_mean, float* running_var, int64_t* num_batches_tracked,
+                        float* scale_shift, float* mean_invstd, void* workspace, int64_t ws_bytes,
+                        hkp_stream_t stream);
+int hkp_bn_stats_seg(int32_t c, int64_t count, int32_t nseg, const int32_t* segments, const float* partials,
+                     double* stats, void* workspace, int64_t ws_bytes, hkp_stream_t stream);
 
 int hkp_bn_stats(int32_t c, int64_t count, int64_t tiles, int32_t tile_rows, const float* partials,
                  double* stats, void* workspace, int64_t ws_bytes, hkp_stream_t stream);
```

Result: faster. 1897 images/sec (median of 6 runs) (+1.3%).
